# qianduoduolr/FGVC

Hardware: AMD Instinct MI355X
Metric: frames/sec + ms/corr-volume, 480p 8-frame clip, 1/2/4/8 MI355X (higher is better)
Workload: dtype f16 + fp6 (e2m3) MFMA operands, f32 accumulate; top-k near-ties re-scored in f64 from f32 features

## Files before the change

fgvc_amd/_lib.py:

```python
from __future__ import annotations

import ctypes as C
import contextlib
import os

_HERE = os.path.dirname(os.path.abspath(__file__))
LIB_PATH = os.environ.get("FGVC_HIP_LIB") or os.path.join(_HERE, "lib", "libfgvc_hip.so")

FGVC_OK = 0
ERR_INVALID_ARG, ERR_UNSUPPORTED, ERR_LAUNCH = 1, 2, 3
NO_LIMIT = 0x3FFFFFFF
PAIR_MASKED = 1
WEIGHT_SOFTMAX, WEIGHT_COSINE, WEIGHT_RAW = 0, 1, 2

_p = C.c_void_p
_i = C.c_int
_f = C.c_float

SIGNATURES = {
    "fgvc_version": (C.c_char_p, []),
    "fgvc_last_error": (C.c_char_p, []),
    "fgvc_set_option": (_i, [C.c_char_p, _i]),
    "fgvc_r2max_for_radius": (_i, [_f]),
    "fgvc_normalize_chw_to_hwc_f32": (_i, [_p, _p, _i, _i, _i, _i, _i, _p]),
    "fgvc_pair_topk_f32": (_i, [_p, _p, _p, _i, _i, _i, _i, _i, _i, _i, _i, _i, _i, _p, _p, _p, _p]),
    "fgvc_pair_topk_f16x3": (_i, [_p, _p, _p, _i, _i, _i, _i, _i, _i, _i, _i, _i, _i, _i, _p, _p, _p]),
    "fgvc_pair_topk_f16x3_runs": (_i, [_p, _p, _p, _i, _i, _i, _i, _i, _i, _i, _i, _i, _i, _i, _p, _i, _p, _p, _p]),
    "fgvc_split_f16x2": (_i, [_p, _p, C.c_int64, _i, _p]),
    "fgvc_split_f16f6p": (_i, [_p, _p, C.c_int64, _i, _p]),
    "fgvc_pair_topk_f16f6": (_i, [_p, _p, _p, _i, _i, _i, _i, _i, _i, _i, _i, _i, _i, _i, _p, _p, _p]),
    "fgvc_pair_topk_f16f6_runs": (_i, [_p, _p, _p, _i, _i, _i, _i, _i, _i, _i, _i, _i, _i, _i, _p, _i, _p, _p, _p]),
    "fgvc_split_f16f6x": (_i, [_p, _p, C.c_int64, _i, _p]),
    "fgvc_pair_topk_f16f6x": (_i, [_p, _p, _p, _i, _i, _i, _i, _i, _i, _i, _i, _i, _i, _i, _p, _p, _p]),
    "fgvc_pair_topk_f16f6x_runs": (_i, [_p, _p, _p, _i, _i, _i, _i, _i, _i, _i, _i, _i, _i, _i, _p, _i, _p, _p, _p]),
    "fgvc_merge_refine_workspace_bytes": (C.c_size_t, [_i, _i]),
    "fgvc_merge_refine_topk_f32": (_i, [_p, _p, _p, _p, _p, C.c_int64, _i, _p, C.c_int64, _i, _i, _i, _i, _i, _i, _i, _i, _i, _f, _i, _f, _i, _i, _i,
                                        _p, _p, _p, _p, _p]),
    "fgvc_pair_topk_f16x3_timed_out": (_i, []),
    "fgvc_pair_topk_f16x3_probe": (_i, [_p]),
    "fgvc_conv64_probe": (_i, [_p]),
    "fgvc_nchw_to_split_nhwc_f32": (_i, [_p, _p, _p, _i, _i, _i, _i, _i, _i, _p]),
    "fgvc_conv_split_f32": (_i, [_p, _p, _p, _p, _p, _p, _i, _i, _i, _i, _i, _i, _i, _i, _i, _p]),
    "fgvc_conv_split_fmt_f32": (_i, [_p, _p, _p, _p, _p, _p, _i, _i, _i, _i, _i, _i, _i, _i, _i, _i, _i, _i, _i, _p, _p]),
    "fgvc_conv_split_proj_fmt_f32": (_i, [_p, _p, _p, _p, _p, _p, _p, _p, _i, _i, _i, _i, _i, _i, _i, _i, _i, _i, _i, _i, _p, _p]),
    "fgvc_conv_split_bank_f16f6p_f32": (_i, [_p, _p, _p, _p, _p, _i, _i, _i, _i, _i, _i, _i, _i, _i, _i, _i, _p]),
    "fgvc_conv_split_bank_f16f6x_f32": (_i, [_p, _p, _p, _p, _p, _i, _i, _i, _i, _i, _i, _i, _i, _i, _i, _i, _p]),
    "fgvc_conv64_split_f32": (_i, [_p, _p, _p, _p, _p, _p, _i, _i, _i, _i, _i, _i, _p]),
    "fgvc_conv64_split_res_f32": (_i, [_p, _p, _p, _p, _p, _p, _p, _i, _i, _i, _i, _i, _i, _p]),
    "fgvc_conv64_split_fmt_f32": (_i, [_p, _p, _p, _p, _p, _p, _p, _i, _i, _i, _i, _i, _i, _i, _i, _i, _i, _p, _p]),
    "fgvc_conv_s2_split_f32": (_i, [_p, _p, _p, _p, _p, _i, _i, _i, _i, _i, _i, _i, _i, _i, _i, _i, _p]),
    "fgvc_conv_s2_split_fmt_f32": (_i, [_p, _p, _p, _p, _p, _i, _i, _i, _i, _i, _i, _i, _i, _i, _i, _i, _i, _i, _p, _p]),
    "fgvc_stem7_split_f32": (_i, [_p, _p, _p, _p, _p, _i, _i, _i, _i, _i, _i, _p]),
    "fgvc_stem7_split_fmt_f32": (_i, [_p, _p, _p, _p, _p, _i, _i, _i, _i, _i, _i, _i, _i, _p, _p]),
    "fgvc_nhwc_to_split_f32": (_i, [_p, _p, _i, _i, _i, _i, _i, _i, _i, _p]),
    "fgvc_normalize_nhwc_f32": (_i, [_p, _p, _i, _i, _i, _i, _i, _p]),
    "fgvc_normalize_split_nhwc_f32": (_i, [_p, _p, _p, _i, _i, _i, _i, _i, _p]),
    "fgvc_normalize_split_f16x2_nhwc_f32": (_i, [_p, _p, _p, _i, _i, _i, _i, _i, _p]),
    "fgvc_normalize_split_f16f6p_nhwc_f32": (_i, [_p, _p, _i, _i, _i, _i, _i, _p]),
    "fgvc_normalize_split_f16f6x_nhwc_f32": (_i, [_p, _p, _i, _i, _i, _i, _i, _p]),
    "fgvc_merge_topk_f32": (_i, [_p, _p, _p, _i, _i, _i, _i, _i, _f, _i, _p, _p, _p, _p]),
    "fgvc_propagate_topk_f32": (_i, [_p, _p, _i, _p, _p, _i, _i, _i, _i, _i, _i, _i, _p, _p]),
    "fgvc_corr_volume_f32": (_i, [_p, _p, _i, _i, _i, _f, _p, _p]),
    "fgvc_split_bf16": (_i, [_p, _p, C.c_int64, _i, _p]),
    "fgvc_corr_volume_bf16x3": (_i, [_p, _p, _i, _i, _i, _f, _p, _p]),
    "fgvc_corr_volume_bf16": (_i, [_p, _p, _i, _i, _i, _f, _p, _p]),
    "fgvc_split_f16f8": (_i, [_p, _p, C.c_int64, _i, _p]),
    "fgvc_corr_volume_f16f8": (_i, [_p, _p, _i, _i, _i, _f, _p, _p]),
    "fgvc_split_f16f6": (_i, [_p, _p, C.c_int64, _i, _p]),
    "fgvc_corr_volume_f16f6": (_i, [_p, _p, _i, _i, _i, _f, _p, _p]),
    "fgvc_debug_store_sweep_f32": (_i, [_p, C.c_int64, _i, _p]),
    "fgvc_dense_attend_splits": (_i, [_i, _i]),
    "fgvc_dense_attend_f32": (_i, [_p, _p, _i, _i, _i, _i, _i, _i, _i, _i, _i, _i, _i, _p, _i, _p]),
    "fgvc_dense_attend_finish_f32": (_i, [_p, _i, _i, _i, _i, _p, _p]),
    "fgvc_dense_kth_f32": (_i, [_p, _i, _i, _i, _p, _i, _p, _p]),
    "fgvc_dense_propagate_f32": (_i, [_p, _p, _i, _i, _i, _p, _p, _i, _p, _p]),
    "fgvc_local_corr_topk_f32": (_i, [_p, _p, _p, _i, _i, _i, _i, _i, _i, _f, _p, _p, _p, _p, _p, _p]),
    "fgvc_local_corr_topk_f16x3": (_i, [_p, _p, _p, _i, _i, _i, _i, _i, _i, _f, _p, _p, _p, _p, _p, _p]),
    "fgvc_local_merge_plan_f32": (_i, [_p, _p, _i, _p, _i, _i, _i, _i, _i, _i, _f, _p, _p, _p, _p]),
    "fgvc_topk_coord_f32": (_i, [_p, _p, _i, _i, _i, _i, _i, _p, _p]),
    "fgvc_topk_coord_rows_f32": (_i, [_p, _p, _i, _i, _i, _i, _i, _i, _p, _p]),
    "fgvc_cycle_chase_f32": (_i, [_p, _p, _p, _i, _i, _i, _i, _i, _p, _p, _p]),
    "fgvc_frames_rgb8_to_lab_f32": (_i, [_p, _i, _i, _i, C.c_int64, C.c_int64, C.c_int64, C.c_int64, _i, _i, _i, _i, _i, _i, _p, _p]),
    "fgvc_jf_tile_rows": (_i, []),
    "fgvc_jf_counts_u8": (_i, [_p, _p, _i, _i, _i, _i, _i, _p, _p]),
    "fgvc_render_frames_u8": (_i, [_p, C.c_int64, C.c_int64, _p, C.c_int64, C.c_int64, _i, _i, _i, _p, C.c_int64, C.c_int64, _p, _i, _i,
                                   _p, C.c_int64, C.c_int64, _p, C.c_int64, C.c_int64, _p, _i, _i, _p, _p]),
    "fgvc_render_tile_rows": (_i, []),
    "fgvc_render_tile_cols": (_i, []),
    "fgvc_c2f_refine_f32": (_i, [_p, _p, _p, _p, _i, _i, _i, _i, _i, _i, _i, _i, _f, _p, _p, _p, _p]),
    "fgvc_c2f_refine_mode_f32": (_i, [_p, _p, _p, _p, _i, _i, _i, _i, _i, _i, _i, _i, _f, _i, _p, _p, _p, _p]),
    "fgvc_bn_act_f32": (_i, [_p, _p, _p, _p, _p, _p, _f, _i, _p, _i, _i, _i, _p]),
    "fgvc_gaussian_labels_f32": (_i, [_p, _i, _i, _i, _i, _f, _p, _p]),
    "fgvc_softargmax_workspace_bytes": (C.c_size_t, [_i, _i]),
    "fgvc_softargmax_top5_f32": (_i, [_p, _i, _i, _i, _i, _i, _i, _p, _f, _p, _p, _p]),
    "fgvc_seg_max_label_u8": (_i, [_p, _i, _i, _i, _i, _p, _p]),
    "fgvc_seg_onehot_labels_u8": (_i, [_p, _i, _i, _i, _i, _i, _p, _p]),
    "fgvc_seg_hard_onehot_f32": (_i, [_p, _i, _i, _p, _p]),
    "fgvc_seg_readout_workspace_bytes": (C.c_size_t, [_i, _i]),
    "fgvc_seg_readout_u8": (_i, [_p, _i, _i, _i, _i, _i, _i, _i, _i, _i, _i, _i, _i, _i, _p, _p, _p]),
    "fgvc_seg_soft_labels_f32": (_i, [_p, _i, _i, _i, _i, _i, _i, _i, _i, _i, _p, _p]),
    "fgvc_seg_soft_labels_f64": (_i, [_p, _i, _i, _i, _i, _i, _i, _i, _i, _i, _p, _p]),
    "fgvc_heatmap_coords_workspace_bytes": (C.c_size_t, [_i, _i]),
    "fgvc_heatmap_coords_f32": (_i, [_p, _p, _i, _i, _i, _i, _i, _i, _i, _i, _i, _i, _i, _i, _i, _i, _p, _p, _p]),
    "fgvc_softmap_readout_f32": (_i, [_p, _p, _i, _i, _i, _i, _i, _i, _i, _i, _i, _i, _i, _i, _i, _i, _i, _i, _p, _p]),
}

_lib = None


class FgvcHipError(RuntimeError):
    pass


def load() -> C.CDLL:
    global _lib
    if _lib is None:
        import torch
        if not os.path.exists(LIB_PATH):
            raise FgvcHipError(
                f"{LIB_PATH} is missing: build it with `python -m fgvc_amd.build` "
                "(hipcc --offload-arch=gfx950). There is no CPU fallback.")
        lib = C.CDLL(LIB_PATH)
        for name, (res, args) in SIGNATURES.items():
            fn = getattr(lib, name)
            fn.restype, fn.argtypes = res, args
        _lib = lib
    return _lib


ABLATIONS_PATH = os.path.join(_HERE, "lib", "libfgvc_hip_ablations.so")
_ablations = None


@contextlib.contextmanager
def ablations():
    global _lib, _ablations
    prod = load()
    if _ablations is None:
        if not os.path.exists(ABLATIONS_PATH):
            raise FgvcHipError(f"{ABLATIONS_PATH} is missing: `python -m fgvc_amd.build` makes it beside the production library")
        lib = C.CDLL(ABLATIONS_PATH)
        for name, (res, args) in SIGNATURES.items():
            fn = getattr(lib, name)
            fn.restype, fn.argtypes = res, args
        _ablations = lib
    _lib = _ablations
    try:
        yield _ablations
    finally:
        _lib = prod


def call(name: str, *args) -> None:
    lib = load()
    rc = getattr(lib, name)(*args)
    if rc != FGVC_OK:
        raise FgvcHipError(f"{name} failed (code {rc}): {lib.fgvc_last_error().decode()}")
```

fgvc_amd/csrc/capi.hip:

```cpp
#include <stdarg.h>
#include <string.h>

#include "common.hpp"

namespace fgvc {

static thread_local char g_err[512] = "";

void set_error(const char* fmt, ...) {
  va_list ap;
  va_start(ap, fmt);
  vsnprintf(g_err, sizeof(g_err), fmt, ap);
  va_end(ap);
}

int pair_topk_launch(const float*, const float*, const int32_t*, int, int, int, int, int, int, int, int, int, int,
                     const uint8_t*, int32_t*, float*, hipStream_t);
int merge_topk_launch(const int32_t*, const float*, const int32_t*, int, int, int, int, int, float, int, int32_t*,
                      float*, float*, hipStream_t);
int normalize_launch(const float*, float*, int, int, int, int, int, hipStream_t);
int propagate_launch(const float*, const int32_t*, int, const int32_t*, const float*, int, int, int, int, int, int,
                     int, float*, hipStream_t);
int bn_act_launch(const float*, const float*, const float*, const float*, const float*, const float*, float, int, float*,
                  int, int, int, hipStream_t);
int gaussian_launch(const float*, int, int, int, int, float, float*, hipStream_t);
int softargmax_launch(const float*, int, int, int, int, int, int, const float*, float, double*, float*, hipStream_t);
int softargmax_bands();
int corr_volume_f32_launch(const float*, const float*, int, int, int, float, float*, hipStream_t);
int split_bf16_launch(const float*, uint16_t*, long long, int, hipStream_t);
int corr_volume_bf16_launch(const uint16_t*, const uint16_t*, int, int, int, float, float*, int, hipStream_t);
int local_merge_launch(const int32_t*, const float*, int, int, int, int, int, float, int32_t*, float*, float*,
                       hipStream_t);
int local_merge_plan_launch(const int32_t*, const float*, const int32_t*, int, int, int, int, int, int, int, float, int32_t*, float*,
                            float*, hipStream_t);
int topk_coord_launch(const int32_t*, const float*, int, int, int, int, int, float*, hipStream_t);
int topk_coord_rows_launch(const int32_t*, const float*, int, int, int, int, int, int, float*, hipStream_t);
int cycle_chase_launch(const float*, const float*, const float*, int, int, int, int, int, float*, float*, hipStream_t);
int frames_rgb8_to_lab_launch(const uint8_t*, int, int, int, long long, long long, long long, long long, int, int, int, int, int, int, float*,
                              hipStream_t);
int jf_counts_launch(const uint8_t*, const uint8_t*, int, int, int, int, int, int64_t*, hipStream_t);
int jf_tile_rows();
int render_frames_launch(const uint8_t*, long long, long long, uint8_t*, long long, long long, int, int, int, const uint8_t*, long long, long long,
                         const uint8_t*, int, int, const double*, long long, long long, const uint8_t*, long long, long long, const uint8_t*, int,
                         int, const double*, hipStream_t);
void render_tile(int*, int*);
int c2f_refine_launch(const int32_t*, const float*, const float*, const float*, int, int, int, int, int, int, int,
                      int, float, int, float*, int32_t*, float*, hipStream_t);

int conv_split_launch(const uint16_t*, const uint16_t*, const float*, const float*, uint16_t*, float*, int, int, int, int, int,
                      int, int, int, int, int, int, int, int, int*, hipStream_t, unsigned char* y_bank = nullptr, int bank_normalize = 1, const uint16_t* x2 = nullptr,
                      const uint16_t* w2 = nullptr, int Cin2 = 0, int bank_row_bytes = 1024);
int conv_s2_launch(const uint16_t*, const uint16_t*, const float*, uint16_t*, float*, int, int, int, int, int, int, int, int, int,
                   int, int, int, int, int*, hipStream_t);
int conv64_launch(const uint16_t*, const uint16_t*, const float*, const float*, const uint16_t*, uint16_t*, float*, int, int, int, int, int, int,
                  int, int, int, int, int*, hipStream_t);
int stem7_launch(const float*, const uint16_t*, const float*, uint16_t*, float*, int, int, int, int, int, int, int, int, int, int, int*,
                 hipStream_t);
int nchw_to_split_nhwc_launch(const float*, uint16_t*, float*, int, int, int, int, int, int, hipStream_t);
int normalize_nhwc_launch(const float*, float*, uint16_t*, int, int, int, int, int, int, hipStream_t);
int nhwc_to_split_launch(float*, uint16_t*, int, int, int, int, int, int, int, hipStream_t);

void set_conv_cot_cap(int);
void set_conv_narrow(int);
void set_conv64_variant(int);
int conv64_probe_read(long long*);
void set_conv_debug(int);
void set_corr6_skew(int);
void set_corr6_sdma(int);
void set_pair_debug(int);
void set_readout_prune(int);
void set_conv_s2_debug(int);
int split_f16x2_launch(const float*, uint16_t*, long long, int, hipStream_t);
int split_f16f6p_launch(const float*, unsigned char*, long long, int, hipStream_t);
int pair_topk_v7_launch(const uint16_t*, const uint16_t*, const int32_t*, int, int, int, int, int, int, int, int, int, const int32_t*, int,
                        int32_t*, float*, int, hipStream_t);
int pair_topk_v5_launch(const uint16_t*, const uint16_t*, const int32_t*, int, int, int, int, int, int, int, int, int, int, const int32_t*,
                        int, int32_t*, float*, hipStream_t);
void set_pair_v5_debug(int);
int pair_v5_timeout_flag();
int pair_v5_probe_read(long long*);
void set_corr_debug(int);
int split_f16f8_launch(const float*, unsigned char*, long long, int, hipStream_t);
int corr_volume_f16f8_launch(const unsigned char*, const unsigned char*, int, int, float, float*, hipStream_t);
void set_corr8_debug(int);
int split_f16f6_launch(const float*, unsigned char*, long long, hipStream_t);
int corr_volume_f16f6_launch(const unsigned char*, const unsigned char*, int, int, float, float*, hipStream_t);
void set_corr6_debug(int);
int store_sweep_launch(float*, long long, int, hipStream_t);
int dense_attend_splits(int, int);
int dense_attend_launch(const float*, const float*, int, int, int, int, int, int, int, int, int, int, int, float*, int, hipStream_t, const float*);
int dense_kth_launch(const float*, int, int, int, float*, int, float*, hipStream_t);
int dense_attend_finish_launch(const float*, int, int, int, int, float*, hipStream_t);

static bool aligned16(const void* p) { return (reinterpret_cast<uintptr_t>(p) & 15u) == 0; }

}

using namespace fgvc;

extern "C" {

const char* fgvc_version(void) { return "fgvc_hip 0.1 (gfx950)"; }
const char* fgvc_last_error(void) { return g_err; }

static int ablation_bits(const char* name, int value) {
  if (strcmp(name, "corr_debug") == 0 || strcmp(name, "pair_debug") == 0 || strcmp(name, "conv_s2_debug") == 0) return value;
  if (strcmp(name, "corr8_debug") == 0) return value & (1 | 2);
  if (strcmp(name, "corr6_debug") == 0) return value & (1 | 2 | 256 | 512 | 1024);
  if (strcmp(name, "conv_debug") == 0) return value & (1 | 2 | 4);
  if (strcmp(name, "pair_f16_debug") == 0)
    return value & ((value & 4194304) ? (1 | 2 | 524288 | 1048576) : (1 | 2 | 4 | 8 | 16 | 32 | 64 | 2048 | 524288 | 1048576));
  return 0;
}

int fgvc_set_option(const char* name, int value) {
  FGVC_REQUIRE(name != nullptr, FGVC_ERR_INVALID_ARG, "fgvc_set_option: null name");
#ifndef FGVC_ABLATIONS
  FGVC_REQUIRE(ablation_bits(name, value) == 0, FGVC_ERR_UNSUPPORTED,
               "fgvc_set_option: %s = %d switches a profiling ablation on (bits %d: results would be wrong); this library is built without them -- "
               "use libfgvc_hip_ablations.so (FGVC_HIP_LIB)", name, value, ablation_bits(name, value));
#endif
  if (strcmp(name, "corr_debug") == 0) {
    set_corr_debug(value);
    return FGVC_OK;
  }
  if (strcmp(name, "corr8_debug") == 0) {
    set_corr8_debug(value);
    return FGVC_OK;
  }
  if (strcmp(name, "corr6_debug") == 0) {
    set_corr6_debug(value);
    return FGVC_OK;
  }
  if (strcmp(name, "pair_debug") == 0) {
    set_pair_debug(value);
    return FGVC_OK;
  }
  if (strcmp(name, "corr6_sdma") == 0) {
    set_corr6_sdma(value);
    return FGVC_OK;
  }
  if (strcmp(name, "corr6_skew") == 0) {
    set_corr6_skew(value);
    return FGVC_OK;
  }
  if (strcmp(name, "conv_debug") == 0) {
    set_conv_debug(value);
    return FGVC_OK;
  }
  if (strcmp(name, "conv64_variant") == 0) {
    set_conv64_variant(value);
    return FGVC_OK;
  }
  if (strcmp(name, "conv_narrow") == 0) {
    set_conv_narrow(value);
    return FGVC_OK;
  }
  if (strcmp(name, "conv_cot_cap") == 0) {
    FGVC_REQUIRE(value == 0 || value == 64 || value == 128, FGVC_ERR_INVALID_ARG, "fgvc_set_option: conv_cot_cap must be 0, 64 or 128");
    set_conv_cot_cap(value);
    return FGVC_OK;
  }
  if (strcmp(name, "pair_f16_debug") == 0) {
    set_pair_v5_debug(value);
    return FGVC_OK;
  }
  if (strcmp(name, "conv_s2_debug") == 0) {
    set_conv_s2_debug(value);
    return FGVC_OK;
  }
  if (strcmp(name, "readout_prune") == 0) {
    set_readout_prune(value != 0);
    return FGVC_OK;
  }
  set_error("fgvc_set_option: unknown option '%s'", name);
  return FGVC_ERR_INVALID_ARG;
}

int fgvc_r2max_for_radius(float radius) {
  if (!(radius > 0.f)) return -1;
  long long d2 = (long long)ceil((double)radius * (double)radius) + 2;
  if (d2 > FGVC_NO_LIMIT) return FGVC_NO_LIMIT;
  while (d2 >= 0 && !(sqrtf((float)d2) < radius)) --d2;
  return (int)d2;
}

int fgvc_normalize_chw_to_hwc_f32(const float* in, float* out, int n, int C, int HW, int normalize, int c_out,
                                  void* stream) {
  FGVC_REQUIRE(in && out, FGVC_ERR_INVALID_ARG, "fgvc_normalize_chw_to_hwc_f32: null pointer");
  FGVC_REQUIRE(n >= 0 && C > 0 && HW > 0, FGVC_ERR_INVALID_ARG, "fgvc_normalize_chw_to_hwc_f32: bad shape n=%d C=%d HW=%d", n, C, HW);
  FGVC_REQUIRE(C <= 1024, FGVC_ERR_UNSUPPORTED, "fgvc_normalize_chw_to_hwc_f32: C=%d > 1024 (LDS tile)", C);
  FGVC_REQUIRE(n <= 65535, FGVC_ERR_UNSUPPORTED, "fgvc_normalize_chw_to_hwc_f32: n=%d > 65535 frames per call", n);
  FGVC_REQUIRE(c_out >= C, FGVC_ERR_INVALID_ARG, "fgvc_normalize_chw_to_hwc_f32: c_out=%d < C=%d", c_out, C);
  if (n == 0) return FGVC_OK;
  return normalize_launch(in, out, n, C, HW, normalize, c_out, (hipStream_t)stream);
}

int fgvc_pair_topk_f32(const float* qfeat, const float* kfeat, const int32_t* pairs, int n_pairs, int C, int Hq,
                       int Wq, int Hk, int Wk, int r2max, int ry, int rx, int topk, const uint8_t* dense_mask,
                       int32_t* idx_out, float* score_out, void* stream) {
  FGVC_REQUIRE(qfeat && kfeat && pairs && idx_out && score_out, FGVC_ERR_INVALID_ARG, "fgvc_pair_topk_f32: null pointer");
  FGVC_REQUIRE(aligned16(qfeat) && aligned16(kfeat) && aligned16(pairs), FGVC_ERR_INVALID_ARG,
               "fgvc_pair_topk_f32: qfeat/kfeat/pairs must be 16-byte aligned");
  FGVC_REQUIRE(Hq > 0 && Wq > 0 && Hk > 0 && Wk > 0 && n_pairs >= 0, FGVC_ERR_INVALID_ARG,
               "fgvc_pair_topk_f32: bad shape Hq=%d Wq=%d Hk=%d Wk=%d n_pairs=%d", Hq, Wq, Hk, Wk, n_pairs);
  FGVC_REQUIRE(topk >= 1 && topk <= 16, FGVC_ERR_UNSUPPORTED, "fgvc_pair_topk_f32: topk=%d outside 1..16", topk);
// ... 468 lines not shown
int fgvc_bn_act_f32(const float* x, const float* residual, const float* mean, const float* var, const float* gamma,
                    const float* beta, float eps, int relu, float* out, int N, int C, int HW, void* stream) {
  FGVC_REQUIRE(x && mean && var && gamma && beta && out, FGVC_ERR_INVALID_ARG, "fgvc_bn_act_f32: null pointer");
  FGVC_REQUIRE(N >= 0 && C > 0 && HW > 0 && eps >= 0.f, FGVC_ERR_INVALID_ARG, "fgvc_bn_act_f32: bad shape");
  if (N == 0) return FGVC_OK;
  return bn_act_launch(x, residual, mean, var, gamma, beta, eps, relu, out, N, C, HW, (hipStream_t)stream);
}

static bool conv_pad_ok(int H, int W, int Hp, int Wp) {
  return Hp >= 8 * cdiv(H, 8) + 2 && Wp >= 32 * cdiv(W, 32) + 8;
}

int fgvc_nchw_to_split_nhwc_f32(const float* in, uint16_t* out, float* out_f32, int N, int C, int H, int W, int Hp, int Wp,
                                void* stream) {
  FGVC_REQUIRE(in && (out || out_f32), FGVC_ERR_INVALID_ARG, "fgvc_nchw_to_split_nhwc_f32: null pointer");
  FGVC_REQUIRE(N >= 0 && C > 0 && C % 32 == 0 && H > 0 && W > 0, FGVC_ERR_INVALID_ARG,
               "fgvc_nchw_to_split_nhwc_f32: bad shape (C must be a multiple of 32)");
  FGVC_REQUIRE(conv_pad_ok(H, W, Hp, Wp), FGVC_ERR_INVALID_ARG,
               "fgvc_nchw_to_split_nhwc_f32: padded size %dx%d too small for %dx%d (need >= 8*ceil(H/8)+2 x 32*ceil(W/32)+8)", Hp, Wp, H, W);
  FGVC_REQUIRE(aligned16(out) && aligned16(out_f32) && (long long)N * (C / 32) <= 65535 && H <= 65535, FGVC_ERR_INVALID_ARG,
               "fgvc_nchw_to_split_nhwc_f32: alignment / grid limits");
  if (N == 0) return FGVC_OK;
  return nchw_to_split_nhwc_launch(in, out, out_f32, N, C, H, W, Hp, Wp, (hipStream_t)stream);
}

int fgvc_conv_split_f32(const uint16_t* x, const uint16_t* w, const float* bias, const float* residual, uint16_t* y_split,
                        float* y_f32, int N, int H, int W, int Hp, int Wp, int Cin, int Cout, int KS, int relu,
                        void* stream) {
  return fgvc_conv_split_fmt_f32(x, w, bias, residual, y_split, y_f32, N, H, W, Hp, Wp, Cin, Cout, KS, relu, FGVC_ACT_BF16X2, 0,
                                 FGVC_ACT_BF16X2, 0, nullptr, stream);
}

int fgvc_conv_split_fmt_f32(const uint16_t* x, const uint16_t* w, const float* bias, const float* residual, uint16_t* y_split,
                            float* y_f32, int N, int H, int W, int Hp, int Wp, int Cin, int Cout, int KS, int relu, int in_fmt,
                            int in_scale_log2, int out_fmt, int out_scale_log2, int* overflow, void* stream) {
  FGVC_REQUIRE(x && w && bias && (y_split || y_f32), FGVC_ERR_INVALID_ARG, "fgvc_conv_split_f32: null pointer");
  FGVC_REQUIRE(in_fmt >= 0 && in_fmt <= 3 && out_fmt >= 0 && out_fmt <= 3, FGVC_ERR_INVALID_ARG, "fgvc_conv_split_fmt_f32: unknown format %d / %d", in_fmt, out_fmt);
  FGVC_REQUIRE(out_fmt == FGVC_ACT_BF16X2 || !y_split || overflow, FGVC_ERR_INVALID_ARG, "fgvc_conv_split_fmt_f32: an f16-format output needs the overflow word");
  FGVC_REQUIRE(in_scale_log2 > -100 && in_scale_log2 < 100 && out_scale_log2 > -100 && out_scale_log2 < 100, FGVC_ERR_INVALID_ARG,
               "fgvc_conv_split_fmt_f32: scale exponent out of range");
  FGVC_REQUIRE(N >= 0 && H > 0 && W > 0, FGVC_ERR_INVALID_ARG, "fgvc_conv_split_f32: bad shape");
  FGVC_REQUIRE(KS == 1 || KS == 3, FGVC_ERR_UNSUPPORTED, "fgvc_conv_split_f32: kernel size %d (1 or 3, stride 1)", KS);
  FGVC_REQUIRE(Cin > 0 && Cin % 32 == 0 && Cout > 0 && Cout % 64 == 0, FGVC_ERR_UNSUPPORTED,
               "fgvc_conv_split_f32: Cin=%d must be a multiple of 32 and Cout=%d of 64", Cin, Cout);
  FGVC_REQUIRE(conv_pad_ok(H, W, Hp, Wp), FGVC_ERR_INVALID_ARG, "fgvc_conv_split_f32: padded size %dx%d too small for %dx%d", Hp, Wp, H, W);
  FGVC_REQUIRE(aligned16(x) && aligned16(w) && aligned16(bias) && aligned16(residual) && aligned16(y_split) && aligned16(y_f32),
               FGVC_ERR_INVALID_ARG, "fgvc_conv_split_f32: 16-byte alignment required");
  FGVC_REQUIRE((const void*)x != (const void*)y_split, FGVC_ERR_INVALID_ARG, "fgvc_conv_split_f32: in-place not supported");
  if (N == 0) return FGVC_OK;
  return conv_split_launch(x, w, bias, residual, y_split, y_f32, N, H, W, Hp, Wp, Cin, Cout, KS, relu, in_fmt, in_scale_log2, out_fmt,
                           out_scale_log2, overflow, (hipStream_t)stream);
}

int fgvc_conv_split_proj_fmt_f32(const uint16_t* x, const uint16_t* w, const uint16_t* x2, const uint16_t* w2, const float* bias,
                                 const float* residual, uint16_t* y_split, float* y_f32, int N, int H, int W, int Hp, int Wp, int Cin, int Cin2,
                                 int relu, int in_fmt, int in_scale_log2, int out_fmt, int out_scale_log2, int* overflow, void* stream) {
  FGVC_REQUIRE(x && w && x2 && w2 && bias && (y_split || y_f32), FGVC_ERR_INVALID_ARG, "fgvc_conv_split_proj_fmt_f32: null pointer");
  FGVC_REQUIRE(in_fmt >= 0 && in_fmt <= 3 && out_fmt >= 0 && out_fmt <= 3, FGVC_ERR_INVALID_ARG, "fgvc_conv_split_proj_fmt_f32: unknown format %d / %d", in_fmt, out_fmt);
  FGVC_REQUIRE(out_fmt == FGVC_ACT_BF16X2 || !y_split || overflow, FGVC_ERR_INVALID_ARG, "fgvc_conv_split_proj_fmt_f32: an f16-format output needs the overflow word");
  FGVC_REQUIRE(in_scale_log2 > -100 && in_scale_log2 < 100 && out_scale_log2 > -100 && out_scale_log2 < 100, FGVC_ERR_INVALID_ARG,
               "fgvc_conv_split_proj_fmt_f32: scale exponent out of range");
  FGVC_REQUIRE(N >= 0 && H > 0 && W > 0, FGVC_ERR_INVALID_ARG, "fgvc_conv_split_proj_fmt_f32: bad shape");
  FGVC_REQUIRE(Cin > 0 && Cin % 32 == 0 && Cin2 > 0 && Cin2 % 32 == 0, FGVC_ERR_UNSUPPORTED,
               "fgvc_conv_split_proj_fmt_f32: Cin=%d and Cin2=%d must be multiples of 32 (Cout is 256)", Cin, Cin2);
  FGVC_REQUIRE(conv_pad_ok(H, W, Hp, Wp), FGVC_ERR_INVALID_ARG, "fgvc_conv_split_proj_fmt_f32: padded size %dx%d too small for %dx%d", Hp, Wp, H, W);
  FGVC_REQUIRE(aligned16(x) && aligned16(w) && aligned16(x2) && aligned16(w2) && aligned16(bias) && aligned16(residual) && aligned16(y_split) &&
               aligned16(y_f32), FGVC_ERR_INVALID_ARG, "fgvc_conv_split_proj_fmt_f32: 16-byte alignment required");
  FGVC_REQUIRE((const void*)x != (const void*)y_split && (const void*)x2 != (const void*)y_split, FGVC_ERR_INVALID_ARG,
               "fgvc_conv_split_proj_fmt_f32: in-place not supported");
  if (N == 0) return FGVC_OK;
  return conv_split_launch(x, w, bias, residual, y_split, y_f32, N, H, W, Hp, Wp, Cin, 256, 3, relu, in_fmt, in_scale_log2, out_fmt,
                           out_scale_log2, overflow, (hipStream_t)stream, nullptr, 1, x2, w2, Cin2);
}

static int conv_split_bank_common(const uint16_t* x, const uint16_t* w, const float* bias, const float* residual, void* bank, int N,
                                  int H, int W, int Hp, int Wp, int Cin, int KS, int relu, int in_fmt, int in_scale_log2,
                                  int normalize, void* stream, int row_bytes) {
  FGVC_REQUIRE(x && w && bias && bank, FGVC_ERR_INVALID_ARG, "fgvc_conv_split_bank_f16f6p_f32: null pointer");
  FGVC_REQUIRE(in_fmt >= 0 && in_fmt <= 3, FGVC_ERR_INVALID_ARG, "fgvc_conv_split_bank_f16f6p_f32: unknown format %d", in_fmt);
  FGVC_REQUIRE(in_scale_log2 > -100 && in_scale_log2 < 100, FGVC_ERR_INVALID_ARG, "fgvc_conv_split_bank_f16f6p_f32: scale exponent out of range");
  FGVC_REQUIRE(N >= 0 && H > 0 && W > 0, FGVC_ERR_INVALID_ARG, "fgvc_conv_split_bank_f16f6p_f32: bad shape");
  FGVC_REQUIRE(KS == 3, FGVC_ERR_UNSUPPORTED, "fgvc_conv_split_bank_f16f6p_f32: kernel size %d (3 x 3, stride 1: the last convolution of a BasicBlock)", KS);
  FGVC_REQUIRE(Cin > 0 && Cin % 32 == 0, FGVC_ERR_UNSUPPORTED, "fgvc_conv_split_bank_f16f6p_f32: Cin=%d must be a multiple of 32 (Cout is 256)", Cin);
  FGVC_REQUIRE(conv_pad_ok(H, W, Hp, Wp), FGVC_ERR_INVALID_ARG, "fgvc_conv_split_bank_f16f6p_f32: padded size %dx%d too small for %dx%d", Hp, Wp, H, W);
  FGVC_REQUIRE(aligned16(x) && aligned16(w) && aligned16(bias) && aligned16(residual) && aligned16(bank), FGVC_ERR_INVALID_ARG,
               "fgvc_conv_split_bank_f16f6p_f32: 16-byte alignment required");
  if (N == 0) return FGVC_OK;
  return conv_split_launch(x, w, bias, residual, nullptr, nullptr, N, H, W, Hp, Wp, Cin, 256, KS, relu, in_fmt, in_scale_log2, 0, 0, nullptr,
                           (hipStream_t)stream, reinterpret_cast<unsigned char*>(bank), normalize, nullptr, nullptr, 0, row_bytes);
}

int fgvc_conv_split_bank_f16f6p_f32(const uint16_t* x, const uint16_t* w, const float* bias, const float* residual, void* bank, int N,
                                    int H, int W, int Hp, int Wp, int Cin, int KS, int relu, int in_fmt, int in_scale_log2,
                                    int normalize, void* stream) {
  return conv_split_bank_common(x, w, bias, residual, bank, N, H, W, Hp, Wp, Cin, KS, relu, in_fmt, in_scale_log2, normalize, stream, 1024);
}

int fgvc_conv_split_bank_f16f6x_f32(const uint16_t* x, const uint16_t* w, const float* bias, const float* residual, void* bank, int N,
                                    int H, int W, int Hp, int Wp, int Cin, int KS, int relu, int in_fmt, int in_scale_log2,
                                    int normalize, void* stream) {
  return conv_split_bank_common(x, w, bias, residual, bank, N, H, W, Hp, Wp, Cin, KS, relu, in_fmt, in_scale_log2, normalize, stream, 2048);
}

int fgvc_conv64_probe(int64_t* out32) {
  FGVC_REQUIRE(out32 != nullptr, FGVC_ERR_INVALID_ARG, "fgvc_conv64_probe: null pointer");
  return conv64_probe_read(reinterpret_cast<long long*>(out32)) == 0 ? FGVC_OK : FGVC_ERR_LAUNCH;
}

int fgvc_conv64_split_f32(const uint16_t* x, const uint16_t* w, const float* bias, const float* residual, uint16_t* y_split,
                          float* y_f32, int N, int H, int W, int Hp, int Wp, int relu, void* stream) {
  return fgvc_conv64_split_res_f32(x, w, bias, residual, nullptr, y_split, y_f32, N, H, W, Hp, Wp, relu, stream);
}

int fgvc_conv64_split_res_f32(const uint16_t* x, const uint16_t* w, const float* bias, const float* residual,
                              const uint16_t* residual_split, uint16_t* y_split, float* y_f32, int N, int H, int W, int Hp, int Wp,
                              int relu, void* stream) {
  return fgvc_conv64_split_fmt_f32(x, w, bias, residual, residual_split, y_split, y_f32, N, H, W, Hp, Wp, relu, FGVC_ACT_BF16X2, 0,
                                   FGVC_ACT_BF16X2, 0, nullptr, stream);
}

int fgvc_conv64_split_fmt_f32(const uint16_t* x, const uint16_t* w, const float* bias, const float* residual,
                              const uint16_t* residual_split, uint16_t* y_split, float* y_f32, int N, int H, int W, int Hp, int Wp,
                              int relu, int in_fmt, int in_scale_log2, int out_fmt, int out_scale_log2, int* overflow, void* stream) {
  FGVC_REQUIRE(x && w && bias && (y_split || y_f32), FGVC_ERR_INVALID_ARG, "fgvc_conv64_split_f32: null pointer");
  FGVC_REQUIRE((in_fmt == FGVC_ACT_BF16X2 || in_fmt == FGVC_ACT_F16F8) && (out_fmt == FGVC_ACT_BF16X2 || out_fmt == FGVC_ACT_F16F8),
               FGVC_ERR_UNSUPPORTED, "fgvc_conv64_split_fmt_f32: formats %d -> %d (bf16x2 or f16f8)", in_fmt, out_fmt);
  FGVC_REQUIRE(out_fmt == FGVC_ACT_BF16X2 || !y_split || overflow, FGVC_ERR_INVALID_ARG,
               "fgvc_conv64_split_fmt_f32: an f16-format output needs the overflow word");
  FGVC_REQUIRE(in_scale_log2 > -100 && in_scale_log2 < 100 && out_scale_log2 > -100 && out_scale_log2 < 100, FGVC_ERR_INVALID_ARG,
               "fgvc_conv64_split_fmt_f32: scale exponent out of range");
  FGVC_REQUIRE(!(residual && residual_split), FGVC_ERR_INVALID_ARG, "fgvc_conv64_split_res_f32: one residual, f32 or split, not both");
  FGVC_REQUIRE(!residual_split || in_fmt == FGVC_ACT_BF16X2, FGVC_ERR_UNSUPPORTED,
               "fgvc_conv64_split_fmt_f32: a split residual is read as (hi, lo) bf16: bf16x2 tensors only");
  FGVC_REQUIRE(N >= 0 && H > 0 && W > 0, FGVC_ERR_INVALID_ARG, "fgvc_conv64_split_f32: bad shape");
  FGVC_REQUIRE(conv_pad_ok(H, W, Hp, Wp), FGVC_ERR_INVALID_ARG, "fgvc_conv64_split_f32: padded size %dx%d too small for %dx%d", Hp, Wp, H, W);
  FGVC_REQUIRE(aligned16(x) && aligned16(w) && aligned16(bias) && aligned16(residual) && aligned16(residual_split) && aligned16(y_split) &&
                   aligned16(y_f32),
               FGVC_ERR_INVALID_ARG, "fgvc_conv64_split_f32: 16-byte alignment required");
  FGVC_REQUIRE((const void*)x != (const void*)y_split && (!residual_split || (const void*)residual_split != (const void*)y_split),
               FGVC_ERR_INVALID_ARG, "fgvc_conv64_split_f32: in-place not supported");
  if (N == 0) return FGVC_OK;
  return conv64_launch(x, w, bias, residual, residual_split, y_split, y_f32, N, H, W, Hp, Wp, relu, in_fmt, in_scale_log2, out_fmt,
                       out_scale_log2, overflow, (hipStream_t)stream);
}

int fgvc_conv_s2_split_f32(const uint16_t* x, const uint16_t* w, const float* bias, uint16_t* y_split, float* y_f32, int N,
                           int H, int W, int Hp, int Wp, int Cin, int Cout, int KS, int Hop, int Wop, int relu, void* stream) {
  return fgvc_conv_s2_split_fmt_f32(x, w, bias, y_split, y_f32, N, H, W, Hp, Wp, Cin, Cout, KS, Hop, Wop, relu, FGVC_ACT_BF16X2, 0, nullptr, stream);
}

int fgvc_conv_s2_split_fmt_f32(const uint16_t* x, const uint16_t* w, const float* bias, uint16_t* y_split, float* y_f32, int N,
                               int H, int W, int Hp, int Wp, int Cin, int Cout, int KS, int Hop, int Wop, int relu, int out_fmt,
                               int out_scale_log2, int* overflow, void* stream) {
  FGVC_REQUIRE(x && w && bias && (y_split || y_f32), FGVC_ERR_INVALID_ARG, "fgvc_conv_s2_split_f32: null pointer");
  FGVC_REQUIRE(out_fmt >= 0 && out_fmt <= 3 && out_scale_log2 > -100 && out_scale_log2 < 100, FGVC_ERR_INVALID_ARG, "fgvc_conv_s2_split_fmt_f32: bad output format / scale");
  FGVC_REQUIRE(out_fmt == FGVC_ACT_BF16X2 || !y_split || overflow, FGVC_ERR_INVALID_ARG, "fgvc_conv_s2_split_fmt_f32: an f16-format output needs the overflow word");
  FGVC_REQUIRE(N >= 0 && H > 0 && W > 0, FGVC_ERR_INVALID_ARG, "fgvc_conv_s2_split_f32: bad shape");
  FGVC_REQUIRE(KS == 1 || KS == 3, FGVC_ERR_UNSUPPORTED, "fgvc_conv_s2_split_f32: kernel size %d (1 or 3, stride 2)", KS);
  FGVC_REQUIRE(Cin > 0 && Cin % 32 == 0 && Cout > 0 && Cout % 32 == 0, FGVC_ERR_UNSUPPORTED,
               "fgvc_conv_s2_split_f32: Cin=%d and Cout=%d must be multiples of 32", Cin, Cout);
  const int Ho = (H - 1) / 2 + 1, Wo = (W - 1) / 2 + 1;
  FGVC_REQUIRE(conv_pad_ok(H, W, Hp, Wp), FGVC_ERR_INVALID_ARG, "fgvc_conv_s2_split_f32: padded size %dx%d too small for %dx%d", Hp, Wp, H, W);
  FGVC_REQUIRE(!y_split || conv_pad_ok(Ho, Wo, Hop, Wop), FGVC_ERR_INVALID_ARG,
               "fgvc_conv_s2_split_f32: padded output size %dx%d too small for %dx%d", Hop, Wop, Ho, Wo);
  FGVC_REQUIRE(aligned16(x) && aligned16(w) && aligned16(bias) && aligned16(y_split) && aligned16(y_f32),
               FGVC_ERR_INVALID_ARG, "fgvc_conv_s2_split_f32: 16-byte alignment required");
  FGVC_REQUIRE((const void*)x != (const void*)y_split, FGVC_ERR_INVALID_ARG, "fgvc_conv_s2_split_f32: in-place not supported");
  if (N == 0) return FGVC_OK;
  return conv_s2_launch(x, w, bias, y_split, y_f32, N, Hp, Wp, Cin, Cout, KS, Ho, Wo, Hop, Wop, relu, out_fmt, out_scale_log2, overflow,
                        (hipStream_t)stream);
}

int fgvc_stem7_split_f32(const float* x, const uint16_t* w, const float* bias, uint16_t* y_split, float* y_f32, int N, int H,
                         int W, int Hop, int Wop, int relu, void* stream) {
  return fgvc_stem7_split_fmt_f32(x, w, bias, y_split, y_f32, N, H, W, Hop, Wop, relu, FGVC_ACT_BF16X2, 0, nullptr, stream);
}

int fgvc_stem7_split_fmt_f32(const float* x, const uint16_t* w, const float* bias, uint16_t* y_split, float* y_f32, int N, int H,
                             int W, int Hop, int Wop, int relu, int out_fmt, int out_scale_log2, int* overflow, void* stream) {
  FGVC_REQUIRE(x && w && bias && (y_split || y_f32), FGVC_ERR_INVALID_ARG, "fgvc_stem7_split_f32: null pointer");
  FGVC_REQUIRE(out_fmt == FGVC_ACT_BF16X2 || out_fmt == FGVC_ACT_F16F8, FGVC_ERR_UNSUPPORTED, "fgvc_stem7_split_fmt_f32: output format %d", out_fmt);
  FGVC_REQUIRE(out_fmt == FGVC_ACT_BF16X2 || !y_split || overflow, FGVC_ERR_INVALID_ARG,
               "fgvc_stem7_split_fmt_f32: an f16-format output needs the overflow word");
  FGVC_REQUIRE(out_scale_log2 > -100 && out_scale_log2 < 100, FGVC_ERR_INVALID_ARG, "fgvc_stem7_split_fmt_f32: scale exponent out of range");
  FGVC_REQUIRE(N >= 0 && H > 0 && W > 0, FGVC_ERR_INVALID_ARG, "fgvc_stem7_split_f32: bad shape");
  const int Ho = (H - 1) / 2 + 1, Wo = (W - 1) / 2 + 1;
  FGVC_REQUIRE(!y_split || conv_pad_ok(Ho, Wo, Hop, Wop), FGVC_ERR_INVALID_ARG,
               "fgvc_stem7_split_f32: padded output size %dx%d too small for %dx%d", Hop, Wop, Ho, Wo);
  FGVC_REQUIRE(aligned16(w) && aligned16(bias) && aligned16(y_split) && aligned16(y_f32) && ((uintptr_t)x & 3) == 0,
               FGVC_ERR_INVALID_ARG, "fgvc_stem7_split_f32: alignment (16 bytes; 4 for x)");
  if (N == 0) return FGVC_OK;
  return stem7_launch(x, w, bias, y_split, y_f32, N, H, W, Ho, Wo, Hop, Wop, relu, out_fmt, out_scale_log2, overflow, (hipStream_t)stream);
}

int fgvc_nhwc_to_split_f32(float* x, uint16_t* out, int N, int C, int H, int W, int Hp, int Wp, int relu, void* stream) {
  FGVC_REQUIRE(x && out, FGVC_ERR_INVALID_ARG, "fgvc_nhwc_to_split_f32: null pointer");
  FGVC_REQUIRE(N >= 0 && C > 0 && C % 32 == 0 && H > 0 && W > 0, FGVC_ERR_INVALID_ARG,
               "fgvc_nhwc_to_split_f32: bad shape (C must be a multiple of 32)");
  FGVC_REQUIRE(conv_pad_ok(H, W, Hp, Wp), FGVC_ERR_INVALID_ARG, "fgvc_nhwc_to_split_f32: padded size %dx%d too small for %dx%d", Hp, Wp, H, W);
  FGVC_REQUIRE(aligned16(x) && aligned16(out), FGVC_ERR_INVALID_ARG, "fgvc_nhwc_to_split_f32: 16-byte alignment required");
  FGVC_REQUIRE((long long)N * H * W * C / 4 < (1ll << 31) * 256, FGVC_ERR_UNSUPPORTED, "fgvc_nhwc_to_split_f32: tensor too large");
  if (N == 0) return FGVC_OK;
  return nhwc_to_split_launch(x, out, N, C, H, W, Hp, Wp, relu, (hipStream_t)stream);
}

static int normalize_split_common(const char* what, const float* in, float* out_f32, uint16_t* out_split, int N, int C, int H, int W,
                                  int normalize, int fmt, void* stream) {
  FGVC_REQUIRE(in && (out_f32 || out_split), FGVC_ERR_INVALID_ARG, "%s: null pointer", what);
  FGVC_REQUIRE(N >= 0 && C > 0 && C % 4 == 0 && H > 0 && W > 0, FGVC_ERR_INVALID_ARG, "%s: bad shape", what);
  FGVC_REQUIRE(aligned16(in) && aligned16(out_f32) && aligned16(out_split), FGVC_ERR_INVALID_ARG, "%s: 16-byte alignment required", what);
  if (N == 0) return FGVC_OK;
  return normalize_nhwc_launch(in, out_f32, out_split, N, C, H, W, normalize, fmt, (hipStream_t)stream);
}

int fgvc_normalize_split_nhwc_f32(const float* in, float* out_f32, uint16_t* out_split, int N, int C, int H, int W, int normalize,
                                  void* stream) {
  return normalize_split_common("fgvc_normalize_split_nhwc_f32", in, out_f32, out_split, N, C, H, W, normalize, 0, stream);
}

int fgvc_normalize_split_f16x2_nhwc_f32(const float* in, float* out_f32, uint16_t* out_split, int N, int C, int H, int W,
                                        int normalize, void* stream) {
  return normalize_split_common("fgvc_normalize_split_f16x2_nhwc_f32", in, out_f32, out_split, N, C, H, W, normalize, 1, stream);
}

int fgvc_normalize_split_f16f6p_nhwc_f32(const float* in, uint8_t* rows, int N, int C, int H, int W, int normalize, void* stream) {
  FGVC_REQUIRE(C == 256, FGVC_ERR_UNSUPPORTED, "fgvc_normalize_split_f16f6p_nhwc_f32: C=%d unsupported (256 only)", C);
  return normalize_split_common("fgvc_normalize_split_f16f6p_nhwc_f32", in, nullptr, reinterpret_cast<uint16_t*>(rows), N, C, H, W, normalize, 2, stream);
}

int fgvc_normalize_split_f16f6x_nhwc_f32(const float* in, uint8_t* rows, int N, int C, int H, int W, int normalize, void* stream) {
  FGVC_REQUIRE(C == 256, FGVC_ERR_UNSUPPORTED, "fgvc_normalize_split_f16f6x_nhwc_f32: C=%d unsupported (256 only)", C);
  return normalize_split_common("fgvc_normalize_split_f16f6x_nhwc_f32", in, nullptr, reinterpret_cast<uint16_t*>(rows), N, C, H, W, normalize, 3, stream);
}

int fgvc_normalize_nhwc_f32(const float* in, float* out, int N, int C, int H, int W, int normalize, void* stream) {
  FGVC_REQUIRE(in && out, FGVC_ERR_INVALID_ARG, "fgvc_normalize_nhwc_f32: null pointer");
  return fgvc_normalize_split_nhwc_f32(in, out, nullptr, N, C, H, W, normalize, stream);
}

int fgvc_gaussian_labels_f32(const float* points, int P, int Hf, int Wf, int stride, float sigma, float* out,
                             void* stream) {
  FGVC_REQUIRE(points && out, FGVC_ERR_INVALID_ARG, "fgvc_gaussian_labels_f32: null pointer");
  FGVC_REQUIRE(P > 0 && Hf > 0 && Wf > 0 && stride >= 1 && sigma > 0.f, FGVC_ERR_INVALID_ARG, "fgvc_gaussian_labels_f32: bad shape");
  return gaussian_launch(points, P, Hf, Wf, stride, sigma, out, (hipStream_t)stream);
}

size_t fgvc_softargmax_workspace_bytes(int n_frames, int P) {
  if (n_frames < 0 || P < 0) return 0;
  return (size_t)n_frames * P * (softargmax_bands() * (2 * 5 + 1) + 1) * sizeof(float);
}

int fgvc_softargmax_top5_f32(const float* labels, int n_frames, int Hf, int Wf, int P, int h, int w,
                             const float* gauss_points, float sigma, double* coords, void* workspace, void* stream) {
  FGVC_REQUIRE(labels && coords, FGVC_ERR_INVALID_ARG, "fgvc_softargmax_top5_f32: null pointer");
  FGVC_REQUIRE(n_frames >= 0 && Hf > 0 && Wf > 0 && P > 0 && h > 0 && w > 0, FGVC_ERR_INVALID_ARG, "fgvc_softargmax_top5_f32: bad shape");
  FGVC_REQUIRE((long long)h * w < (1ll << 31) && h * w >= 5, FGVC_ERR_UNSUPPORTED, "fgvc_softargmax_top5_f32: h*w out of range");
  FGVC_REQUIRE(n_frames <= 65535 && sigma > 0.f, FGVC_ERR_INVALID_ARG, "fgvc_softargmax_top5_f32: bad n_frames/sigma");
  FGVC_REQUIRE(workspace != nullptr || n_frames == 0, FGVC_ERR_INVALID_ARG,
               "fgvc_softargmax_top5_f32: workspace of fgvc_softargmax_workspace_bytes() bytes required");
  FGVC_REQUIRE(P <= 65535, FGVC_ERR_UNSUPPORTED, "fgvc_softargmax_top5_f32: P > 65535");
  if (n_frames == 0) return FGVC_OK;
  return softargmax_launch(labels, n_frames, Hf, Wf, P, h, w, gauss_points, sigma, coords,
                           static_cast<float*>(workspace), (hipStream_t)stream);
}

}
```

fgvc_amd/csrc/conv_s2.hip:

```cpp
#include "common.hpp"

namespace fgvc {

struct ConvS2Params {
  const uint16_t* x;
  const uint16_t* w;
  const float* bias;
  uint16_t* y_split;
  float* y_f32;
  int N, Hp, Wp, Cin, Cout, Ho, Wo, Hop, Wop, relu;
  int n_ty, n_tx;
  int debug;
  float out_scale;
  int out_fmt;
  int* overflow;
};


__device__ __forceinline__ void s2_lds_dma_16(const void* src_lane, uint32_t lds_uniform) {
  asm volatile("s_mov_b32 m0, %1\n\ts_nop 0\n\tglobal_load_lds_dwordx4 %0, off" ::"v"(src_lane), "s"(lds_uniform) : "memory");
}
__device__ __forceinline__ uint32_t s2_lds_addr(const void* p) {
  return (uint32_t)(size_t)(const __attribute__((address_space(3))) unsigned char*)p;
}
__device__ __forceinline__ int s2_swz(int e, int s) { return e * 128 + ((s ^ ((e >> 1) & 7)) << 4); }

constexpr int S2_TR = 4;
constexpr int S2_NW = 2 * S2_TR;
constexpr int S2_CPG = 1;
constexpr int S2_RS = 144;

template <int KS>
__global__ __launch_bounds__(64 * S2_NW, 2) void conv_s2_kernel(ConvS2Params p) {
  constexpr int T = KS * KS;
  constexpr int NR = KS == 3 ? 2 * S2_TR + 1 : S2_TR;
  constexpr int NC = KS == 3 ? 65 : 32;
  constexpr int NE = NR * NC;
  constexpr int NG = (NE + 7) / 8;
  constexpr int CHUNKB = NG * 8 * 128;
  constexpr int SMEMB = S2_CPG * CHUNKB > S2_NW * 32 * S2_RS ? S2_CPG * CHUNKB : S2_NW * 32 * S2_RS;
  static_assert(SMEMB <= 79 * 1024, "LDS: two workgroups per CU");
  __shared__ __attribute__((aligned(16))) unsigned char smem[SMEMB];
  auto wave_sync = [&]() { asm volatile("s_waitcnt lgkmcnt(0)" ::: "memory"); };

  const int tid = threadIdx.x, lane = tid & 63;
  const int wave = __builtin_amdgcn_readfirstlane(tid >> 6);
  const int ct = wave & 3, half = wave >> 2;
  const int n = lane & 31, h = lane >> 5;
  int bid = blockIdx.x;
  const int nimg = bid / (p.n_ty * p.n_tx);
  bid -= nimg * p.n_ty * p.n_tx;
  const int ty = bid / p.n_tx, tx = bid - ty * p.n_tx;
  const int y0 = ty * S2_TR, x0 = tx * 32;
  const int co_w = blockIdx.y * 128 + ct * 32;
  const bool active = co_w < p.Cout;
  const int nchunk = p.Cin / 32;
  const size_t pix_bytes_in = (size_t)nchunk * 128;
  const int d_row = lane >> 3, d_slot = lane & 7;

  f32x16 acc[2];
#pragma unroll
  for (int b = 0; b < 2; ++b)
#pragma unroll
    for (int r = 0; r < 16; ++r) acc[b][r] = 0.f;

  const int n_ct = p.Cout / 32;
  const uint16_t* wlane = p.w + (size_t)(active ? (co_w >> 5) : 0) * 2048 + lane * 8;
  f32x4 bias_v[4];
#pragma unroll
  for (int g = 0; g < 4; ++g) bias_v[g] = *reinterpret_cast<const f32x4*>(p.bias + (active ? co_w : 0) + 8 * g + 4 * h);

  for (int cg = 0; cg < nchunk; cg += S2_CPG) {
    const int ncg = imin(S2_CPG, nchunk - cg);
    for (int i = wave; i < ((p.debug & 1) ? 0 : ncg * NG); i += S2_NW) {
      const int cc = i / NG, g = i - cc * NG;
      const int e = imin(g * 8 + d_row, NE - 1);
      const int j = e / NC, m = e - j * NC;
      int prow, pcol;
      if (KS == 3) {
        prow = 2 * y0 + j;
        pcol = 2 * x0 + (m < 33 ? 2 * m : 2 * (m - 33) + 1);
      } else {
        prow = 2 * (y0 + j) + 1;
        pcol = 2 * (x0 + m) + 1;
      }
      if (prow >= p.Hp || pcol >= p.Wp) prow = pcol = 0;
      const int sl = d_slot ^ ((e >> 1) & 7);
      const unsigned char* src = reinterpret_cast<const unsigned char*>(p.x) +
                                 (((size_t)nimg * p.Hp + prow) * p.Wp + pcol) * pix_bytes_in + (size_t)(cg + cc) * 128 + sl * 16;
      s2_lds_dma_16(src, s2_lds_addr(smem + cc * CHUNKB + g * 1024));
    }
    asm volatile("s_waitcnt vmcnt(0)" ::: "memory");
    __syncthreads();

    const int nit = ncg * T;
    bf16x8 a_cur[4], a_nxt[4];
    auto load_a = [&](bf16x8* a, int it) {
      const int cc = it / T, t = it - cc * T;
      const uint16_t* wp = wlane + ((size_t)t * nchunk + (cg + cc)) * n_ct * 2048;
#pragma unroll
      for (int q = 0; q < 4; ++q) a[q] = *reinterpret_cast<const bf16x8*>((p.debug & 8) ? wlane + q * 512 : wp + q * 512);
    };
    load_a(a_cur, 0);
    for (int it = 0; it < nit; ++it) {
      if (it + 1 < nit) load_a(a_nxt, it + 1);
      __builtin_amdgcn_sched_barrier(0);
      const int cc = it / T, t = it - cc * T;
      const int dy = KS == 3 ? t / 3 : 0, dx = KS == 3 ? t - 3 * (t / 3) : 0;
      const int mbase = KS == 3 ? (dx == 0 ? 0 : dx == 1 ? 33 : 1) : 0;
      const unsigned char* patch = smem + cc * CHUNKB;
#pragma unroll
      for (int b = 0; b < 2; ++b) {
        const int r = half * 2 + b;
        const int e = (KS == 3 ? (2 * r + dy) : r) * NC + mbase + n;
        bf16x8 xh[2], xl[2];
#pragma unroll
        for (int s = 0; s < 2; ++s) {
          xh[s] = *reinterpret_cast<const bf16x8*>(patch + s2_swz(e, 2 * s + h));
          xl[s] = *reinterpret_cast<const bf16x8*>(patch + s2_swz(e, 4 + 2 * s + h));
        }
        if (p.debug & 2) {
          acc[b][0] += (float)(xh[0][0] + xl[0][0] + xh[1][0] + xl[1][0] + a_cur[0][0] + a_cur[1][0] + a_cur[2][0] + a_cur[3][0]);
          continue;
        }
#pragma unroll
        for (int s = 0; s < 2; ++s) {
          acc[b] = __builtin_amdgcn_mfma_f32_32x32x16_bf16(a_cur[s], xh[s], acc[b], 0, 0, 0);
          acc[b] = __builtin_amdgcn_mfma_f32_32x32x16_bf16(a_cur[2 + s], xh[s], acc[b], 0, 0, 0);
          acc[b] = __builtin_amdgcn_mfma_f32_32x32x16_bf16(a_cur[s], xl[s], acc[b], 0, 0, 0);
        }
      }
#pragma unroll
      for (int q = 0; q < 4; ++q) a_cur[q] = a_nxt[q];
    }
    __syncthreads();
  }
  if (!active || (p.debug & 4)) return;

  unsigned char* tile = smem + wave * (32 * S2_RS);
  const int mv_row = lane >> 3, mv_col = (lane & 7) * 16;
#pragma unroll
  for (int b = 0; b < 2; ++b) {
    const int y = y0 + half * 2 + b;
    if (y >= p.Ho) continue;
    f32x4 v[4];
#pragma unroll
    for (int g = 0; g < 4; ++g) {
      const f32x4 bv = bias_v[g];
      v[g] = {acc[b][4 * g + 0] + bv.x, acc[b][4 * g + 1] + bv.y, acc[b][4 * g + 2] + bv.z, acc[b][4 * g + 3] + bv.w};
      if (p.relu) {
        v[g].x = fmaxf(v[g].x, 0.f); v[g].y = fmaxf(v[g].y, 0.f); v[g].z = fmaxf(v[g].z, 0.f); v[g].w = fmaxf(v[g].w, 0.f);
      }
    }
    if (p.y_f32) {
#pragma unroll
      for (int g = 0; g < 4; ++g) *reinterpret_cast<f32x4*>(tile + n * S2_RS + (8 * g + 4 * h) * 4) = v[g];
      wave_sync();
      unsigned char* dst = reinterpret_cast<unsigned char*>(p.y_f32 + (((size_t)nimg * p.Ho + y) * p.Wo + x0) * p.Cout + co_w);
#pragma unroll
      for (int i = 0; i < 4; ++i) {
        const int row = i * 8 + mv_row;
        if (x0 + row < p.Wo)
          *reinterpret_cast<uint4*>(dst + (size_t)row * p.Cout * 4 + mv_col) =
              *reinterpret_cast<const uint4*>(tile + row * S2_RS + mv_col);
      }
      wave_sync();
    }
    if (p.y_split) {
      if (p.out_fmt == 0) {
#pragma unroll
        for (int g = 0; g < 4; ++g) {
          const f32x4 x = v[g];
          ushort4 hv, lv;
          split_bf16_4(x, hv, lv);
          unsigned char* o = tile + n * S2_RS + (8 * g + 4 * h) * 2;
          *reinterpret_cast<ushort4*>(o) = hv;
          *reinterpret_cast<ushort4*>(o + 64) = lv;
        }
      } else if (p.out_fmt == 3) {
        bool ovf = false;
        uint2 hw[4];
        fgvc_i32x4 main6, tail6;
        split_f16f6_chunk(v, p.out_scale, h, hw, main6, tail6, ovf);
        unsigned char* o = tile + n * S2_RS;
#pragma unroll
        for (int g = 0; g < 4; ++g) *reinterpret_cast<uint2*>(o + (8 * g + 4 * h) * 2) = hw[g];
        *reinterpret_cast<fgvc_i32x4*>(o + 80 - 16 * h) = main6;
        *reinterpret_cast<fgvc_i32x4*>(o + 112 - 16 * h) = tail6;
        if (__builtin_amdgcn_ballot_w64(ovf && x0 + n < p.Wo) != 0ull && lane == 0) atomicOr(p.overflow, 1);
      } else {
        bool ovf = false;
#pragma unroll
        for (int g = 0; g < 4; ++g) {
          uint2 hw, lw;
          uint32_t l8, h8;
          split_f16_4(v[g], p.out_scale, hw, l8, h8, lw, ovf);
          unsigned char* o = tile + n * S2_RS;
          *reinterpret_cast<uint2*>(o + (8 * g + 4 * h) * 2) = hw;
          if (p.out_fmt == 1) {
            *reinterpret_cast<uint32_t*>(o + 64 + 8 * g + 4 * h) = l8;
            *reinterpret_cast<uint32_t*>(o + 96 + 8 * g + 4 * h) = h8;
          } else {
            *reinterpret_cast<uint2*>(o + 64 + (8 * g + 4 * h) * 2) = lw;
          }
        }
        if (__builtin_amdgcn_ballot_w64(ovf && x0 + n < p.Wo) != 0ull && lane == 0) atomicOr(p.overflow, 1);
      }
      wave_sync();
      const size_t pix0 = ((size_t)nimg * p.Hop + (y + 1)) * p.Wop + (x0 + 1);
      unsigned char* dst = reinterpret_cast<unsigned char*>(p.y_split) + (pix0 * (p.Cout / 32) + (co_w >> 5)) * 128;
#pragma unroll
      for (int i = 0; i < 4; ++i) {
        const int row = i * 8 + mv_row;
        if (x0 + row < p.Wo)
          *reinterpret_cast<uint4*>(dst + (size_t)row * p.Cout * 4 + mv_col) =
              *reinterpret_cast<const uint4*>(tile + row * S2_RS + mv_col);
      }
      wave_sync();
    }
  }
}

static int g_conv_s2_debug = 0;
void set_conv_s2_debug(int v) { g_conv_s2_debug = v; }

int conv_s2_launch(const uint16_t* x, const uint16_t* w, const float* bias, uint16_t* y_split, float* y_f32, int N, int Hp,
                   int Wp, int Cin, int Cout, int KS, int Ho, int Wo, int Hop, int Wop, int relu, int out_fmt, int out_scale_log2,
                   int* overflow, hipStream_t s) {
  ConvS2Params p;
  p.out_fmt = out_fmt; p.out_scale = ldexpf(1.0f, out_scale_log2); p.overflow = overflow;
  p.x = x; p.w = w; p.bias = bias; p.y_split = y_split; p.y_f32 = y_f32;
  p.N = N; p.Hp = Hp; p.Wp = Wp; p.Cin = Cin; p.Cout = Cout; p.Ho = Ho; p.Wo = Wo; p.Hop = Hop; p.Wop = Wop; p.relu = relu;
  p.n_ty = cdiv(Ho, S2_TR); p.n_tx = cdiv(Wo, 32);
  p.debug = g_conv_s2_debug;
  dim3 grid(p.n_ty * p.n_tx * N, cdiv(Cout, 128));
  if (KS == 3) conv_s2_kernel<3><<<grid, 64 * S2_NW, 0, s>>>(p);
  else conv_s2_kernel<1><<<grid, 64 * S2_NW, 0, s>>>(p);
  FGVC_CHECK_LAUNCH("fgvc_conv_s2_split_f32");
  return FGVC_OK;
}

}
```

fgvc_amd/mmpt_api/backbones.py:

```python
from __future__ import annotations

import re
from typing import Sequence

import torch
import torch.nn as nn
import torch.nn.functional as F

from .registry import BACKBONES

_CAPTURING = [False]


class ConvBN(nn.Module):

    def __init__(self, cin, cout, k, stride=1, padding=0, dilation=1, relu=True):
        super().__init__()
        self.conv = nn.Conv2d(cin, cout, k, stride, padding, dilation, bias=False)
        self.bn = nn.BatchNorm2d(cout)
        self.relu = relu

    def forward(self, x, residual=None, relu=None):
        relu = self.relu if relu is None else relu
        y = self.conv(x)
        if y.is_cuda and not self.training and y.dtype == torch.float32 and y.is_contiguous():
            from .. import ops
            return ops.bn_act(y, self.bn, residual, relu, inplace=True)
        y = self.bn(y)
        if residual is not None:
            y = y + residual
        return F.relu(y, inplace=True) if relu else y


class BasicBlock(nn.Module):
    expansion = 1

    def __init__(self, cin, planes, stride=1, dilation=1, downsample=None):
        super().__init__()
        self.conv1 = ConvBN(cin, planes, 3, stride, dilation, dilation, relu=True)
        self.conv2 = ConvBN(planes, planes, 3, 1, 1, 1, relu=False)
        self.downsample = downsample

    def forward(self, x):
        idt = x if self.downsample is None else self.downsample(x)
        return self.conv2(self.conv1(x), residual=idt, relu=True)


class Bottleneck(nn.Module):
    expansion = 4

    def __init__(self, cin, planes, stride=1, dilation=1, downsample=None):
        super().__init__()
        self.conv1 = ConvBN(cin, planes, 1, 1, 0, 1, relu=True)
        self.conv2 = ConvBN(planes, planes, 3, stride, dilation, dilation, relu=True)
        self.conv3 = ConvBN(planes, planes * 4, 1, 1, 0, 1, relu=False)
        self.downsample = downsample

    def forward(self, x):
        idt = x if self.downsample is None else self.downsample(x)
        return self.conv3(self.conv2(self.conv1(x)), residual=idt, relu=True)


def _stage(block, cin, planes, n, stride, dilation):
    ds = None
    if stride != 1 or cin != planes * block.expansion:
        ds = ConvBN(cin, planes * block.expansion, 1, stride, 0, 1, relu=False)
    first_dil = dilation if dilation == 1 else dilation // 2
    layers = [block(cin, planes, stride, first_dil, ds)]
    layers += [block(planes * block.expansion, planes, 1, dilation) for _ in range(1, n)]
    return nn.Sequential(*layers)


@BACKBONES.register_module()
class ResNet(nn.Module):
    arch_settings = {18: (BasicBlock, (2, 2, 2, 2)), 34: (BasicBlock, (3, 4, 6, 3)),
                     50: (Bottleneck, (3, 4, 6, 3)), 101: (Bottleneck, (3, 4, 23, 3)),
                     152: (Bottleneck, (3, 8, 36, 3))}

    def __init__(self, depth, pretrained=None, torchvision_pretrain=True, in_channels=3, num_stages=4,
                 strides=(1, 2, 2, 2), dilations=(1, 1, 1, 1), out_indices=(3,), planes_custom=None,
                 pool_type="max", zero_init_residual=True, **unused):
        super().__init__()
        if depth not in self.arch_settings:
            raise KeyError(f"invalid depth {depth} for resnet")
        assert 1 <= num_stages <= 4 and len(strides) == len(dilations) == num_stages
        assert max(out_indices) < num_stages
        self.depth, self.pretrained, self.torchvision_pretrain = depth, pretrained, torchvision_pretrain
        self.strides, self.dilations, self.out_indices = tuple(strides), tuple(dilations), tuple(out_indices)
        self.zero_init_residual = zero_init_residual
        block, counts = self.arch_settings[depth]
        self.conv1 = ConvBN(in_channels, 64, 7, 2, 3, 1, relu=True)
        self.pool = {"max": nn.MaxPool2d(3, 2, 1), "mean": nn.AvgPool2d(3, 2, 1)}.get(pool_type)
        cin = 64
        self.res_layers = []
        for i, n in enumerate(counts[:num_stages]):
            planes = planes_custom[i] if planes_custom is not None else 64 * 2 ** i
            self.add_module(f"layer{i + 1}", _stage(block, cin, planes, n, strides[i], dilations[i]))
            self.res_layers.append(f"layer{i + 1}")
            cin = planes * block.expansion
        self.feat_dim = cin

    def init_weights(self):
        self.reset_split_cache()
        if isinstance(self.pretrained, (str, dict)):
            if self.torchvision_pretrain:
                load_torchvision_checkpoint(self, self.pretrained)
            elif isinstance(self.pretrained, str):
                load_checkpoint(self, self.pretrained)
            else:
                raise Exception("a state dict is only accepted as a torchvision checkpoint (resnet.py:590)")
            return
        for m in self.modules():
            if isinstance(m, nn.Conv2d):
                nn.init.kaiming_normal_(m.weight, mode="fan_out", nonlinearity="relu")
            elif isinstance(m, nn.BatchNorm2d):
                nn.init.constant_(m.weight, 1)
                nn.init.constant_(m.bias, 0)
        if self.zero_init_residual:
            for m in self.modules():
                if isinstance(m, BasicBlock):
                    nn.init.constant_(m.conv2.bn.weight, 0)
                elif isinstance(m, Bottleneck):
                    nn.init.constant_(m.conv3.bn.weight, 0)

    use_conv64 = True
    use_stem7 = True
    use_s2_conv = True
    conv64_f16f8 = True
    res_from_split = False
    use_split_conv = True
    arith = "f16f6"
    fold_projection = True
    layer1_whole_batch = True
    fuse_bank = True

    @staticmethod
    def supported_arith():
        return ("f16f6", "f16f8", "bf16x3", "f16x3")

    def set_arith(self, arith: str):
        if arith not in self.supported_arith():
            raise ValueError(f"arith={arith!r}: one of {self.supported_arith()}")
        if arith != self.arith:
            self.arith = arith
            self.reset_split_cache()

    def _generic_s1(self, cb) -> bool:
        c = cb.conv
        return c.stride == (1, 1) and not (self.use_conv64 and tuple(c.weight.shape) == (64, 64, 3, 3))

    def _is_conv64(self, cb) -> bool:
        c = cb.conv
        return bool(self.use_conv64 and c.stride == (1, 1) and tuple(c.weight.shape) == (64, 64, 3, 3))

    def _stem7_ok(self) -> bool:
        c1 = self.conv1.conv
        return bool(self.use_stem7 and c1.kernel_size == (7, 7) and c1.stride == (2, 2) and c1.padding == (3, 3) and c1.in_channels == 3
                    and c1.out_channels == 64 and c1.dilation == (1, 1) and self.conv1.relu)

    def _format_plan(self, last: int):
        from .. import ops
        fmt, bf = ops.ACT_FMT[self.arith], ops.ACT_BF16X2
        cache = self.__dict__.setdefault("_split_cache", {})
        key = ("fmt_plan", self.arith, last, self.use_conv64, self.use_s2_conv, self.use_stem7, self.conv64_f16f8)
        if key not in cache:
            blocks = [(s_i, b_i, blk) for s_i in range(last + 1) for b_i, blk in enumerate(getattr(self, self.res_layers[s_i]))]
            f64 = ops.ACT_F16F8 if (fmt in (ops.ACT_F16F8, ops.ACT_F16F6) and self.conv64_f16f8) else bf

            def reads(cb):
                if self._is_conv64(cb):
                    return f64
                return fmt if self._generic_s1(cb) else bf

            def can_write(cb, f):
                if f == bf:
                    return True
                if self._is_conv64(cb):
                    return f == ops.ACT_F16F8
                return self._generic_s1(cb) or (cb.conv.stride == (2, 2) and self.use_s2_conv)

            def wants(blk):
                f = reads(blk.conv1)
                return f if (blk.downsample is None or reads(blk.downsample) == f) else bf
            plan = {}
            f_in = wants(blocks[0][2]) if blocks else bf
            if f_in != bf and not (self._stem7_ok() and f_in == ops.ACT_F16F8):
                f_in = bf
            plan["stem"] = f_in
            for i, (s_i, b_i, blk) in enumerate(blocks):
                f_a = reads(blk.conv2) if can_write(blk.conv1, reads(blk.conv2)) else bf
                nxt = blocks[i + 1][2] if i + 1 < len(blocks) else None
                f_y = wants(nxt) if (nxt is not None and can_write(blk.conv2, wants(nxt))) else bf
                plan[(s_i, b_i)] = (f_in, f_a, f_y)
                f_in = f_y
            cache[key] = plan
        return cache[key]

    def _block_formats(self, si: int, bi: int, last: int):
        return self._format_plan(last)[(si, bi)]


    def _projection_fold(self, blk, wt, si, bi, dev, f_in, f_a, s_in, s_a, Cout, banked):
        from .. import ops
        ds, c2 = blk.downsample, blk.conv2
        if not (self.fold_projection and not banked and f_in == f_a and f_a != ops.ACT_F16F8 and wt["c2"][3] == "s1" and wt["ds"] is not None
                and wt["ds"][3] == "s1" and Cout == 256 and c2.conv.kernel_size == (3, 3) and ds.conv.kernel_size == (1, 1)
                and ds.conv.stride == (1, 1) and ds.conv.in_channels % 32 == 0):
            return None
        cache = self.__dict__.setdefault("_split_cache", {})
        e = s_a + wt["c2"][2] - s_in
        key = ("wproj", si, bi, dev, self.arith, f_a, e)
        if key not in cache:
            w = ds.conv.weight.detach()
            if f_a == ops.ACT_BF16X2:
                w2, b2 = ops.prepare_conv_split(w, ds.bn)
            else:
                sc = (ds.bn.weight / torch.sqrt(ds.bn.running_var + ds.bn.eps)).detach().float().abs().view(-1, 1, 1, 1)
                top = float((w.detach().float().abs() * sc).max()) * 2.0 ** e
                if not (2.0 ** -6 <= top < 2.0 ** 14) and top != 0.0:
                    cache[key] = None
                    return None
                w2, b2, _ = ops.prepare_conv_split_f16(w, ds.bn, f_a, force_exp=e)
            cache[key] = (w2, (wt["c2"][1] + b2).contiguous())
        return cache[key]

    def _identity_from_split(self, blk) -> bool:
        c2 = getattr(blk, "conv2", None)
        return bool(self.use_conv64 and self.res_from_split and not (self.arith in ("f16f8", "f16f6") and self.conv64_f16f8)
                    and isinstance(blk, BasicBlock) and blk.downsample is None
                    and c2 is not None and tuple(c2.conv.weight.shape) == (64, 64, 3, 3) and c2.conv.stride == (1, 1)
                    and tuple(blk.conv1.conv.weight.shape) == (64, 64, 3, 3) and blk.conv1.conv.stride == (1, 1))

    def _scales(self, dev):
        cache = self.__dict__.setdefault("_split_cache", {})
        return cache.get(("scales", dev))

    calibration = "canonical"
    CANON_TARGET_LOG2 = 8

    @staticmethod
    def canonical_frames(device):
        g = torch.Generator().manual_seed(0x5CA1E)
        base = torch.randn(2, 3, 24, 24, generator=g)
        x = F.interpolate(base, size=(192, 192), mode="bilinear", align_corners=False) * 1.5 + 0.4 * torch.randn(2, 3, 192, 192, generator=g)
        return x.clamp_(-2.7, 2.7).to(device)

    def calibrate(self, x=None, last=None, device=None):
        from .. import ops
        cache = self.__dict__.setdefault("_split_cache", {})
        canonical = x is None
        if canonical:
            x = self.canonical_frames(device if device is not None else next(self.parameters()).device)
        dev = x.device
        saved = (self.arith, self.split_lanes)
        rec = {}
        self.__dict__["_calib"] = rec
        try:
            self.arith, self.split_lanes = "bf16x3", 1
            self._trunk(x, max(self.out_indices) if last is None else last)
            torch.cuda.synchronize(dev)
        finally:
            self.arith, self.split_lanes = saved
            self.__dict__.pop("_calib", None)
        target = (self.CANON_TARGET_LOG2 if canonical else ops.F16_TARGET_LOG2) - int(self.__dict__.get("_headroom_extra", 0))
        scales = {k: ops.act_scale_log2(float(v), target) for k, v in rec.items()}
        cache[("scales", dev)] = scales
        cache[("scales_from", dev)] = "canonical" if canonical else "frames"
        self._drop_graphs(dev)
        if ("overflow", dev) not in cache:
            cache[("overflow", dev)] = torch.zeros(1, dtype=torch.int32, device=dev)
        self._cache_filled(dev)
        return scales

    def check_overflow(self):
        cache = self.__dict__.get("_split_cache", {})
        hit = False
        for k in [k for k in cache if isinstance(k, tuple) and k and k[0] == "overflow"]:
            if int(cache[k].item()) != 0:
                hit = True
                cache[k].zero_()
                cache.pop(("scales", k[1]), None)
                self._drop_graphs(k[1])
        if hit and self.calibration == "canonical":
            self.__dict__["_headroom_extra"] = min(int(self.__dict__.get("_headroom_extra", 0)) + 4, 12)
        return hit
# ... 13 lines not shown
            if shape_sig is not None and not (k[1][0] == shape_sig[0] and tuple(k[1][2:]) == tuple(shape_sig[1:3]) and k[2] == shape_sig[3]):
                continue
            del cache[k]

    def _load_from_state_dict(self, *args, **kwargs):
        self.__dict__.pop("_split_cache", None)
        return super()._load_from_state_dict(*args, **kwargs)

    def reset_split_cache(self):
        self.__dict__.pop("_split_cache", None)

    def _split_stage_ok(self, stage, x) -> bool:
        if not (self.use_split_conv and x.is_cuda and not self.training and x.dtype == torch.float32):
            return False
        for bi, blk in enumerate(stage):
            if not isinstance(blk, BasicBlock):
                return False
            convs = [blk.conv1.conv, blk.conv2.conv] + ([blk.downsample.conv] if blk.downsample is not None else [])
            for c in convs:
                if (c.dilation != (1, 1) or c.groups != 1 or c.in_channels % 32 or c.out_channels % 64
                        or c.kernel_size not in ((1, 1), (3, 3))):
                    return False
            strided = blk.conv1.conv.stride != (1, 1)
            if blk.conv2.conv.stride != (1, 1) or (strided and (bi > 0 or blk.downsample is None)):
                return False
            if blk.downsample is not None and blk.downsample.conv.stride != blk.conv1.conv.stride:
                return False
            if blk.downsample is None and blk.conv1.conv.in_channels != blk.conv2.conv.out_channels:
                return False
        return True

    def _split_buffers(self, key, N, C, H, W, device, names):
        from .. import ops
        cache = self.__dict__.setdefault("_split_cache", {})
        k = ("b", self.__dict__.get("_ws_sig")) + key + (N, C, H, W, device)
        mk = {"s": ops.alloc_split_nhwc, "f": ops.alloc_nhwc}
        if k not in cache:
            cache[k] = {}
        missing = [nm for nm in names if nm not in cache[k]]
        if missing:
            for nm in missing:
                cache[k][nm] = mk[nm[0]](N, C, H, W, device)
            self._cache_filled(device)
        return cache[k]

    max_workspace_shapes = 2

    def _touch_workspace_shape(self, sig):
        cache = self.__dict__.setdefault("_split_cache", {})
        order = cache.setdefault("_ws_order", [])
        if sig in order:
            order.remove(sig)
        order.append(sig)
        while len(order) > max(1, int(self.max_workspace_shapes)):
            old = order.pop(0)
            if _CAPTURING[0]:
                raise RuntimeError("ResNet: a workspace eviction inside a HIP-graph capture (the graph would keep freed addresses)")
            if isinstance(sig[-1], torch.device) and sig[-1].type == "cuda":
                torch.cuda.synchronize(sig[-1])
            self._drop_graphs(shape_sig=old)
            for k in [k for k in cache if isinstance(k, tuple) and len(k) > 1 and k[0] == "b" and k[1] == old]:
                del cache[k]
        self.__dict__["_ws_sig"] = sig

    @staticmethod
    def _cache_filled(device):
        if _CAPTURING[0]:
            raise RuntimeError("ResNet: a cache entry was made inside a HIP-graph capture (the capture call must find everything in place)")
        torch.cuda.synchronize(device)

    @staticmethod
    def _fold(cb: "ConvBN"):
        bn = cb.bn
        scale = (bn.weight / torch.sqrt(bn.running_var + bn.eps)).detach()
        w = (cb.conv.weight.detach() * scale.view(-1, 1, 1, 1)).contiguous(memory_format=torch.channels_last)
        return w, (bn.bias - bn.running_mean * scale).detach().contiguous()

    def _miopen_nhwc(self, key, cb: "ConvBN", x_cl):
        cache = self.__dict__.setdefault("_split_cache", {})
        k = ("m",) + key + (x_cl.device,)
        if k not in cache:
            cache[k] = self._fold(cb)
            self._cache_filled(x_cl.device)
        w, b = cache[k]
        c = cb.conv
        y = F.conv2d(x_cl, w, b, c.stride, c.padding, c.dilation, c.groups)
        y = y.contiguous(memory_format=torch.channels_last)
        return y.permute(0, 2, 3, 1)

    split_lanes = 2

    def _stage_split(self, si: int, cur, call):
        from .. import ops
        stage = getattr(self, self.res_layers[si])
        cache = self.__dict__.setdefault("_split_cache", {})
        dev = cur["split"].device
        lo, hi, N = cur["lo"], cur["hi"], cur["N"]
        from ..ops import ACT_BF16X2
        last_stage = call["last"]
        fmts = [self._block_formats(si, bi, last_stage) for bi in range(len(stage))]
        calib = self.__dict__.get("_calib")
        scales = self._scales(dev) or {}
        ovf = cache.get(("overflow", dev))
        wkey = ("w", si, dev, self.arith)
        if wkey not in cache:
            def prep_s1(w, bn, fmt):
                if self.use_conv64 and tuple(w.shape) == (64, 64, 3, 3):
                    if fmt == ops.ACT_F16F8:
                        return ops.prepare_conv64_f16(w, bn) + ("conv64",)
                    assert fmt == ACT_BF16X2
                    return ops.prepare_conv64(w, bn) + (0, "conv64")
                if fmt == ACT_BF16X2:
                    return ops.prepare_conv_split(w, bn) + (0, "s1")
                return ops.prepare_conv_split_f16(w, bn, fmt) + ("s1",)

            def prep(cb, fmt):
                st = cb.conv.stride
                if st == (1, 1):
                    return prep_s1(cb.conv.weight.detach(), cb.bn, fmt)
                if st == (2, 2):
                    return ops.prepare_conv_s2(cb.conv.weight.detach(), cb.bn) + (0, "s2")
                return None
            cache[wkey] = [dict(c1=prep(b.conv1, f[0]), c2=prep(b.conv2, f[1]),
                                ds=None if b.downsample is None else prep(b.downsample, f[0]))
                           for b, f in zip(stage, fmts)]
            self._cache_filled(dev)
        full = None
        for bi, (blk, wt) in enumerate(zip(stage, cache[wkey])):
            Cout = blk.conv2.conv.out_channels
            idt_split = None
            H, W = cur["H"], cur["W"]
            f_in, f_a, f_y = fmts[bi]
            s_in = cur.get("scale", 0)
            s_a = scales.get((si, bi, "a"), 0) if f_a != ACT_BF16X2 else 0
            s_y = scales.get((si, bi, "y"), 0) if f_y != ACT_BF16X2 else 0
            assert cur.get("fmt", ACT_BF16X2) == f_in, "split activation format mismatch between producer and consumer"

            def conv_s1(x_split, wb, in_fmt=ACT_BF16X2, in_scale=0, out_fmt=ACT_BF16X2, out_scale=0, **kw):
                if wb[3] == "conv64":
                    ops.conv64_split(x_split, wb[0], wb[1], H, W, in_fmt=in_fmt, in_scale_log2=in_scale + wb[2], out_fmt=out_fmt,
                                     out_scale_log2=out_scale, overflow=ovf, **kw)
                else:
                    ops.conv_split(x_split, wb[0], wb[1], H, W, in_fmt=in_fmt, in_scale_log2=in_scale + wb[2], out_fmt=out_fmt,
                                   out_scale_log2=out_scale, overflow=ovf, **kw)

            last_conv = bi == len(stage) - 1 and not cur["need_split"]
            proj = None
            x_in_split = cur["split"]
            if blk.conv1.conv.stride == (2, 2) and self.use_s2_conv:
                Hi, Wi = H, W
                H, W = (Hi - 1) // 2 + 1, (Wi - 1) // 2 + 1
                bufs = self._split_buffers((si, bi), N, Cout, H, W, dev, ("s_a", "s_y", "f_y", "f_idt"))
                buf = {k: v[lo:hi] for k, v in bufs.items()}
                ops.conv_s2_split(cur["split"], wt["ds"][0], wt["ds"][1], Hi, Wi, relu=False, out_f32=buf["f_idt"])
                idt = buf["f_idt"]
                ops.conv_s2_split(cur["split"], wt["c1"][0], wt["c1"][1], Hi, Wi, relu=True, out_split=buf["s_a"], out_fmt=f_a,
                                  out_scale_log2=s_a, overflow=ovf)
            elif blk.conv1.conv.stride != (1, 1):
                x_cl = cur["f32"].permute(0, 3, 1, 2)
                t1 = self._miopen_nhwc((si, bi, "c1"), blk.conv1, x_cl)
                idt = self._miopen_nhwc((si, bi, "ds"), blk.downsample, x_cl)
                _, H, W, _ = t1.shape
                bufs = self._split_buffers((si, bi), N, Cout, H, W, dev, ("s_a", "s_y", "f_y"))
                buf = {k: v[lo:hi] for k, v in bufs.items()}
                assert f_a == ACT_BF16X2
                ops.nhwc_to_split(t1, buf["s_a"], relu=True)
            else:
                bufs = self._split_buffers((si, bi), N, Cout, H, W, dev, ("s_a", "s_y", "f_y", "f_idt"))
                buf = {k: v[lo:hi] for k, v in bufs.items()}
                if blk.downsample is not None:
                    proj = self._projection_fold(blk, wt, si, bi, dev, f_in, f_a, s_in, s_a, Cout, last_conv and si == call["last"] and call.get("bank_of") is not None)
                if proj is not None:
                    idt = None
                elif blk.downsample is not None:
                    conv_s1(cur["split"], wt["ds"], f_in, s_in, relu=False, out_f32=buf["f_idt"])
                    idt = buf["f_idt"]
                elif self._identity_from_split(blk):
                    idt, idt_split = None, cur["split"]
                else:
                    idt = cur["f32"]
                    assert idt is not None
                conv_s1(cur["split"], wt["c1"], f_in, s_in, f_a, s_a, relu=True, out_split=buf["s_a"])
            if calib is not None:
                calib[(si, bi, "a")] = torch.maximum(calib.get((si, bi, "a"), torch.zeros((), device=dev)),
                                                     buf["s_a"].view(torch.bfloat16)[..., :32].abs().amax().float())
            full = bufs["f_y"]
            if bi == len(stage) - 1 and si in call["fresh"]:
                if si not in call["out"]:
                    with torch.cuda.stream(call["main"]):
                        call["out"][si] = ops.alloc_nhwc(N, Cout, H, W, dev)
                    for st in call["streams"]:
                        if st is not call["main"]:
                            st.wait_stream(call["main"])
                full = call["out"][si]
            f_y_ = full[lo:hi]
            skip_f32 = (not cur["need_f32"]) if bi == len(stage) - 1 else self._identity_from_split(stage[bi + 1])
            if skip_f32:
                f_y_ = None
            kw_res = dict(residual_split=idt_split) if idt_split is not None else dict(residual=idt)
            bank = None
            if (last_conv and si == call["last"] and call.get("bank_of") is not None and wt["c2"][3] == "s1" and Cout == 256
                    and blk.conv2.conv.kernel_size == (3, 3) and idt_split is None and calib is None):
                bank = call["bank_of"](lo, hi, Cout, H, W)
            if bank is not None:
                ops.conv_split_to_bank(buf["s_a"], wt["c2"][0], wt["c2"][1], H, W, True, bank, residual=idt, in_fmt=f_a,
                                       in_scale_log2=s_a + wt["c2"][2], normalize=call["bank_normalize"])
                cur = dict(cur, split=None, f32=None, H=H, W=W, fmt=f_y, scale=s_y, banked=True)
                continue
            if proj is not None:
                ops.conv_split(buf["s_a"], wt["c2"][0], proj[1], H, W, True, out_split=None if last_conv else buf["s_y"], out_f32=f_y_,
                               in_fmt=f_a, in_scale_log2=s_a + wt["c2"][2], out_fmt=f_y, out_scale_log2=s_y, overflow=ovf,
                               x2_split=x_in_split, w2=proj[0])
            else:
                conv_s1(buf["s_a"], wt["c2"], f_a, s_a, f_y, s_y, relu=True, out_split=None if last_conv else buf["s_y"], out_f32=f_y_, **kw_res)
            if calib is not None and not last_conv:
                calib[(si, bi, "y")] = torch.maximum(calib.get((si, bi, "y"), torch.zeros((), device=dev)),
                                                     buf["s_y"].view(torch.bfloat16)[..., :32].abs().amax().float())
            cur = dict(cur, split=buf["s_y"], f32=f_y_, H=H, W=W, fmt=f_y, scale=s_y)
        cur["full"] = full
        return cur

    def _trunk(self, x, last: int, fresh=(), post=None, bank_of=None, bank_normalize=True):
        from .. import ops
        stages = [getattr(self, nm) for nm in self.res_layers[:last + 1]]
        probe = x
        if (self.pool is None and x.is_cuda and x.dtype == torch.float32 and self.conv1.conv.out_channels % 32 == 0
                and all(self._split_stage_ok(st, probe) for st in stages)):
            N, dev = x.shape[0], x.device
            cache = self.__dict__.setdefault("_split_cache", {})
            if self.arith != "bf16x3" and self._scales(dev) is None and "_calib" not in self.__dict__:
                self.calibrate(None if self.calibration == "canonical" else x, last, device=dev)
            self._touch_workspace_shape((N, x.shape[2], x.shape[3], dev))
            n_lanes = 1 if N <= 2 else max(1, min(int(self.split_lanes), N))
            main = torch.cuda.current_stream(dev)
            c1 = self.conv1.conv
            stem7 = None
            f_stem = self._format_plan(last)["stem"]
            s_stem = (self._scales(dev) or {}).get(("stem",), 0) if f_stem != ops.ACT_BF16X2 else 0
            calib = self.__dict__.get("_calib")
            if self._stem7_ok():
                if ("stem7", dev) not in cache:
                    cache[("stem7", dev)] = ops.prepare_stem7(c1.weight.detach(), self.conv1.bn)
                    self._cache_filled(dev)
                stem7 = cache[("stem7", dev)]
                x = x.contiguous()
            x_cl = None if stem7 else x.contiguous(memory_format=torch.channels_last)
            if n_lanes > 1:
                skey = ("streams", dev, n_lanes)
                if skey not in cache:
                    cache[skey] = [torch.cuda.Stream(dev, priority=int(getattr(self, "lane_priority", 0))) for _ in range(n_lanes)]
                streams = cache[skey]
                for s in streams:
                    s.wait_stream(main)
            else:
                streams = [main]
            whole = bool(n_lanes > 1 and self.layer1_whole_batch and last >= 1 and calib is None and 0 not in fresh
                         and all(self._is_conv64(b.conv1) and self._is_conv64(b.conv2) for b in stages[0]))
            lane_streams = [main] if whole else streams
            lanes = []
            for li, s in enumerate(lane_streams):
                lo, hi = (0, N) if whole else (li * N // n_lanes, (li + 1) * N // n_lanes)
                with torch.cuda.stream(s):
                    if stem7:
                        H, W, C0 = (x.shape[2] - 1) // 2 + 1, (x.shape[3] - 1) // 2 + 1, 64
                        if self._identity_from_split(stages[0][0]):
                            sb = self._split_buffers(("stem",), N, C0, H, W, dev, ("s_x",))
                            t = None
                        else:
                            sb = self._split_buffers(("stem",), N, C0, H, W, dev, ("s_x", "f_x"))
                            t = sb["f_x"][lo:hi]
                        ops.stem7_split(x[lo:hi], stem7[0], stem7[1], True, out_split=sb["s_x"][lo:hi], out_f32=t, out_fmt=f_stem,
                                        out_scale_log2=s_stem, overflow=cache.get(("overflow", dev)))
                    else:
                        assert f_stem == ops.ACT_BF16X2
                        t = self._miopen_nhwc(("stem",), self.conv1, x_cl[lo:hi])
                        _, H, W, C0 = t.shape
                        sb = self._split_buffers(("stem",), N, C0, H, W, dev, ("s_x",))
                        ops.nhwc_to_split(t, sb["s_x"][lo:hi], relu=True)
                    if calib is not None:
                        calib[("stem",)] = torch.maximum(calib.get(("stem",), torch.zeros((), device=dev)),
                                                         sb["s_x"][lo:hi].view(torch.bfloat16)[..., :32].abs().amax().float())
                lanes.append(dict(split=sb["s_x"][lo:hi], f32=t, H=H, W=W, lo=lo, hi=hi, N=N, need_split=True, fmt=f_stem, scale=s_stem))
            fulls = []
            call = dict(main=main, streams=streams, fresh=tuple(fresh), out={}, last=last, bank_of=bank_of, bank_normalize=bool(bank_normalize))
            for i in range(last + 1):
                need_f32 = True
                if i < last and i not in call["fresh"]:
                    nb = stages[i + 1][0]
                    st = nb.conv1.conv.stride
                    need_f32 = nb.downsample is None or not (st == (1, 1) or (st == (2, 2) and self.use_s2_conv))
                if whole and i == 0:
                    one = self._stage_split(0, dict(lanes[0], need_split=True, need_f32=need_f32), call)
                    fulls.append(one["full"])
                    for s in streams:
                        s.wait_stream(main)
                    lanes = []
                    for li in range(n_lanes):
                        lo, hi = li * N // n_lanes, (li + 1) * N // n_lanes
                        lanes.append(dict(one, split=one["split"][lo:hi], f32=None if one["f32"] is None else one["f32"][lo:hi], lo=lo, hi=hi))
                    continue
                for li, s in enumerate(streams):
                    with torch.cuda.stream(s):
                        lanes[li] = self._stage_split(i, dict(lanes[li], need_split=i < last, need_f32=need_f32), call)
                fulls.append(lanes[0]["full"])
            if post is not None:
                for ln, s in zip(lanes, streams):
                    if ln.get("banked"):
                        continue
                    with torch.cuda.stream(s):
                        post(ln["f32"], ln["lo"], ln["hi"], ln["f32"].shape[-1], ln["H"], ln["W"])
            if n_lanes > 1:
                for s in streams:
                    main.wait_stream(s)
            outs = [f.permute(0, 3, 1, 2) for f in fulls]
            return outs[:-1], fulls[-1], True, lanes[0]["H"], lanes[0]["W"]
        x = self.conv1(x)
        if self.pool is not None:
            x = self.pool(x)
        outs = []
        for st in stages:
            x = st(x)
            outs.append(x)
        return outs[:-1], x, False, x.shape[-2], x.shape[-1]

    def forward(self, x, out_idx=None):
        want = tuple(out_idx) if out_idx is not None else self.out_indices
        last = max(want)
        earlier, y, nhwc, H, W = self._trunk(x, last, fresh=want)
        if nhwc:
            y = y.permute(0, 3, 1, 2)
        stage_out = earlier + [y]
        outs = [stage_out[i] for i in want]
        return outs[0] if len(outs) == 1 else tuple(outs)

    use_graph = "auto"
    graph_auto_max_px = 300_000

    def forward_hwc(self, x, normalize: bool = True, split_if=None, split_fmt: str = "bf16", out=None):
        want = self.use_graph is True or (self.use_graph == "auto" and x.dim() == 4 and x.shape[0] * x.shape[2] * x.shape[3] <= self.graph_auto_max_px)
        if not (want and x.is_cuda and not self.training and x.dtype == torch.float32) or torch.cuda.is_current_stream_capturing():
            return self.forward_hwc_eager(x, normalize, split_if, split_fmt, out)
        cache = self.__dict__.setdefault("_split_cache", {})
        sig = (self.arith, self.split_lanes, self.use_conv64, self.use_stem7, self.use_s2_conv, self.conv64_f16f8, self.res_from_split,
               self.use_split_conv, self.fuse_bank, self.fold_projection, self.layer1_whole_batch, tuple(self.out_indices))
        key = ("graph", tuple(x.shape), x.device, bool(normalize), split_fmt, split_if is not None, sig)
        ent = cache.get(key)
        if ent is None:
            cache[key] = "warm"
            return self.forward_hwc_eager(x, normalize, split_if, split_fmt, out)
        if ent == "warm":
            if self._scales(x.device) is None and self.arith != "bf16x3":
                return self.forward_hwc_eager(x, normalize, split_if, split_fmt, out)
            static_in = torch.empty_like(x)
            static_in.copy_(x)
            self.forward_hwc_eager(static_in, normalize, split_if, split_fmt, None)
            torch.cuda.synchronize(x.device)
            g = torch.cuda.CUDAGraph()
            _CAPTURING[0] = True
            try:
                with torch.cuda.graph(g):
                    o, H, W = self.forward_hwc_eager(static_in, normalize, split_if, split_fmt, None)
            finally:
                _CAPTURING[0] = False
            ent = cache[key] = (g, static_in, o, H, W)
        g, static_in, o, H, W = ent
        static_in.copy_(x)
        g.replay()
        if out is not None and tuple(out.shape) == tuple(o.shape) and out.dtype == o.dtype:
            out.copy_(o)
            return out, H, W
        return o.clone(), H, W

    def forward_hwc_eager(self, x, normalize: bool = True, split_if=None, split_fmt: str = "bf16", out=None):
        from .. import ops
        assert len(self.out_indices) == 1
        box = {}

        def ensure_out(C, H, W):
            if "out" not in box:
                as_split = bool(split_if is not None and split_if(C, H, W))
                shape = (x.shape[0], H * W, 4 if split_fmt == "f16f6x" else 2, C) if as_split else (x.shape[0], H * W, C)
                dtype = torch.int16 if as_split else torch.float32
                if out is not None and tuple(out.shape) == shape and out.dtype == dtype and out.is_contiguous() and out.device == x.device:
                    box["out"] = out
                else:
                    with torch.cuda.stream(main):
                        box["out"] = torch.empty(shape, device=x.device, dtype=dtype)
                torch.cuda.current_stream(x.device).wait_stream(main)
                box["split"] = as_split
            elif torch.cuda.current_stream(x.device) != main:
                torch.cuda.current_stream(x.device).wait_stream(main)

        def post(y_slice, lo, hi, C, H, W):
            ensure_out(C, H, W)
            ops.normalize_nhwc(y_slice, normalize, split=split_fmt if box["split"] else False, out=box["out"][lo:hi])

        def bank_of(lo, hi, C, H, W):
            if not (self.fuse_bank and split_fmt in ("f16f6", "f16f6x") and C == 256 and split_if is not None and split_if(C, H, W)):
                return None
            ensure_out(C, H, W)
            return box["out"][lo:hi] if box["split"] else None

        main = torch.cuda.current_stream(x.device) if x.is_cuda else None
        _, y, nhwc, H, W = self._trunk(x, self.out_indices[0], post=post, bank_of=bank_of, bank_normalize=normalize)
        if nhwc:
            return box["out"], H, W
        C = y.shape[1]
        as_split = bool(split_if is not None and split_if(C, H, W))
        f = ops.normalize_to_hwc(y.float(), normalize, pad=True)
        splitter = {"f16": ops.split_f16x2, "f16f6": ops.split_f16f6p, "f16f6x": ops.split_f16f6x}.get(split_fmt, ops.split_bf16)
        return (splitter(f) if as_split and f.shape[-1] == C else f), H, W


def torchvision_key(name: str) -> str:
    mod, _, leaf = name.rpartition(".")
    owner, _, part = mod.rpartition(".")
    if part not in ("conv", "bn"):
        return name
    if "downsample" in owner:
        return f"{owner}.{0 if part == 'conv' else 1}.{leaf}"
    return f"{owner if part == 'conv' else owner.replace('conv', 'bn')}.{leaf}"


def load_torchvision_checkpoint(module: nn.Module, filename_or_state):
    sd = torch.load(filename_or_state, map_location="cpu") if isinstance(filename_or_state, str) else filename_or_state
    if isinstance(sd, dict) and "state_dict" in sd:
        sd = sd["state_dict"]
    own = module.state_dict()
    used = set()
    with torch.no_grad():
        for k, v in own.items():
            tv = torchvision_key(k)
            if tv in sd:
                v.copy_(sd[tv])
                used.add(tv)
            elif not k.endswith("num_batches_tracked"):
                raise KeyError(f"torchvision checkpoint has no '{tv}' (for '{k}')")
    if hasattr(module, "reset_split_cache"):
        module.reset_split_cache()
    return sorted(set(sd) - used)


_PREFIXES = (r"^module\.", r"^backbone\.", r"^encoder\.", r"^backbone_fine\.")


def load_checkpoint(module: nn.Module, filename_or_state, strict: bool = False, prefixes: Sequence[str] = _PREFIXES):
    sd = torch.load(filename_or_state, map_location="cpu") if isinstance(filename_or_state, str) else filename_or_state
    if isinstance(sd, dict) and "state_dict" in sd:
        sd = sd["state_dict"]
    own = module.state_dict()
    out = {}
    for k, v in sd.items():
        kk = k
        if kk not in own:
            for p in prefixes:
                k2 = re.sub(p, "", kk)
                if k2 != kk and (k2 in own or not strict):
                    kk = k2
                    if kk in own:
                        break
        out[kk] = v
    return module.load_state_dict({k: v for k, v in out.items() if k in own} if not strict else out, strict=strict)
```

fgvc_amd/ops.py:

```python
from __future__ import annotations

import ctypes as C
import functools
import math
from dataclasses import dataclass
from typing import Optional, Tuple

import torch

from . import _lib
from ._lib import NO_LIMIT, PAIR_MASKED, WEIGHT_COSINE, WEIGHT_RAW, WEIGHT_SOFTMAX


@dataclass(frozen=True)
class MaskSpec:
    r2max: int = NO_LIMIT
    ry: int = NO_LIMIT
    rx: int = NO_LIMIT

    @property
    def is_none(self) -> bool:
        return self.r2max >= NO_LIMIT and self.ry >= NO_LIMIT and self.rx >= NO_LIMIT

    @staticmethod
# ... 718 lines not shown
        return packed, bias, e
    if fmt == ACT_F16F6:
        return _f16f6_slots(h, l, "h").contiguous().view(torch.int16), bias, e
    h8 = (h.float() * 2.0 ** -F8_AW).clamp(-448.0, 448.0).to(torch.float8_e4m3fn)
    l8 = (l * 2.0 ** F8_BW).clamp(-448.0, 448.0).to(torch.float8_e4m3fn)
    packed = torch.cat([h.contiguous().view(torch.uint8), h8.view(torch.uint8), l8.view(torch.uint8)], dim=-1).contiguous()
    return packed.view(torch.int16), bias, e


def prepare_conv64(weight: torch.Tensor, bn: "torch.nn.BatchNorm2d") -> Tuple[torch.Tensor, torch.Tensor]:
    assert tuple(weight.shape) == (64, 64, 3, 3)
    packed, bias = prepare_conv_split(weight, bn)
    v = packed.view(9, 2, 2, 32, 2, 2, 2, 8)
    v = v.permute(2, 0, 1, 5, 4, 6, 3, 7).contiguous()
    return v.view(2, 9, 2, 2, 2, 64, 8), bias


def prepare_conv64_f16(weight: torch.Tensor, bn: "torch.nn.BatchNorm2d") -> Tuple[torch.Tensor, torch.Tensor, int]:
    assert tuple(weight.shape) == (64, 64, 3, 3)
    packed, bias, e = prepare_conv_split_f16(weight, bn, ACT_F16F8)
    rows = packed.view(torch.uint8).view(9, 2, 2, 32, 128)
    hpart = rows[..., :64].reshape(9, 2, 2, 32, 2, 2, 16)
    f16 = hpart.permute(2, 0, 1, 4, 5, 3, 6)
    h8 = rows[..., 64:96].reshape(9, 2, 2, 32, 2, 16)
    l8 = rows[..., 96:128].reshape(9, 2, 2, 32, 2, 16)
    x = torch.stack([h8, l8], dim=-2).permute(2, 0, 1, 4, 3, 5, 6)
    out = torch.cat([f16.reshape(2, 9, 2, 2048), x.reshape(2, 9, 2, 2048)], dim=-1).contiguous()
    return out.view(torch.int16), bias, e


def prepare_conv_s2(weight: torch.Tensor, bn: "torch.nn.BatchNorm2d") -> Tuple[torch.Tensor, torch.Tensor]:
    packed, bias = prepare_conv_split(weight, bn)
    T, nch, Cout, _ = packed.shape
    assert Cout % 32 == 0
    v = packed.view(T, nch, Cout // 32, 32, 2, 2, 2, 8)
    v = v.permute(0, 1, 2, 4, 5, 6, 3, 7).contiguous()
    return v.view(T, nch, Cout // 32, 4, 64, 8), bias


def prepare_stem7(weight: torch.Tensor, bn: "torch.nn.BatchNorm2d") -> Tuple[torch.Tensor, torch.Tensor]:
    Cout, Cin, KS, _ = weight.shape
    assert (Cout, Cin, KS) == (64, 3, 7)
    scale = (bn.weight / torch.sqrt(bn.running_var + bn.eps)).float()
    w = weight.float() * scale.view(-1, 1, 1, 1)
    bias = (bn.bias - bn.running_mean * scale).float().contiguous()
    k = torch.zeros((Cout, 7, 8, 4), device=w.device, dtype=torch.float32)
    k[:, :, :7, :3] = w.permute(0, 2, 3, 1)
    k = k.reshape(2, 32, 7, 2, 2, 8)
    k = k.permute(2, 3, 0, 4, 1, 5).contiguous()
    hi, lo = _split_pair(k)
    packed = torch.stack([hi, lo], dim=3).contiguous()
    return packed.view(torch.int16).view(7, 2, 2, 2, 64, 8), bias


def alloc_split_nhwc(N: int, C: int, H: int, W: int, device) -> torch.Tensor:
    Hp, Wp = conv_pad_dims(H, W)
    return torch.zeros((N, Hp, Wp, C // 32, 64), device=device, dtype=torch.int16)


def alloc_nhwc(N: int, C: int, H: int, W: int, device) -> torch.Tensor:
    return torch.empty((N, H, W, C), device=device, dtype=torch.float32)


def nhwc_to_split(x: torch.Tensor, out: torch.Tensor, relu: bool = False) -> torch.Tensor:
    x = _chk(x, torch.float32, "x")
    N, H, W, C = x.shape
    Hp, Wp = conv_pad_dims(H, W)
    assert out.shape == (N, Hp, Wp, C // 32, 64) and out.dtype == torch.int16 and out.is_contiguous()
    _lib.call("fgvc_nhwc_to_split_f32", _ptr(x), _ptr(out), N, C, H, W, Hp, Wp, int(relu), _stream(x))
    return out


def nchw_to_split_nhwc(x: torch.Tensor, out: Optional[torch.Tensor] = None, out_f32: Optional[torch.Tensor] = None,
                       want_split: bool = True) -> Optional[torch.Tensor]:
    x = _chk(x, torch.float32, "x")
    N, C, H, W = x.shape
    if out is None and want_split:
        out = alloc_split_nhwc(N, C, H, W, x.device)
    Hp, Wp = conv_pad_dims(H, W)
    if out is not None:
        assert out.shape == (N, Hp, Wp, C // 32, 64) and out.dtype == torch.int16 and out.is_contiguous()
    if out_f32 is not None:
        assert out_f32.shape == (N, H, W, C) and out_f32.dtype == torch.float32 and out_f32.is_contiguous()
    _lib.call("fgvc_nchw_to_split_nhwc_f32", _ptr(x), _ptr(out), _ptr(out_f32), N, C, H, W, Hp, Wp, _stream(x))
    return out


def conv_split(x_split: torch.Tensor, w: torch.Tensor, bias: torch.Tensor, H: int, W: int, relu: bool,
               residual: Optional[torch.Tensor] = None, out_split: Optional[torch.Tensor] = None,
               out_f32: Optional[torch.Tensor] = None, in_fmt: int = ACT_BF16X2, in_scale_log2: int = 0,
               out_fmt: int = ACT_BF16X2, out_scale_log2: int = 0, overflow: Optional[torch.Tensor] = None,
               x2_split: Optional[torch.Tensor] = None, w2: Optional[torch.Tensor] = None) -> None:
    x_split, w = _chk(x_split, torch.int16, "x_split"), _chk(w, torch.int16, "w")
    bias = _chk(bias, torch.float32, "bias")
    N, Hp, Wp, nch, _ = x_split.shape
    taps, nch_w, Cout, _ = w.shape
    assert nch_w == nch and taps in (1, 9) and bias.shape == (Cout,)
    for t, dt, shape in ((residual, torch.float32, (N, H, W, Cout)), (out_f32, torch.float32, (N, H, W, Cout)),
                         (out_split, torch.int16, (N, Hp, Wp, Cout // 32, 64))):
        if t is not None:
            assert t.dtype == dt and tuple(t.shape) == shape and t.is_contiguous() and t.device == x_split.device, "conv_split buffer"
    if out_fmt != ACT_BF16X2 and out_split is not None:
        assert overflow is not None and overflow.dtype == torch.int32 and overflow.device == x_split.device
    if x2_split is not None:
        x2_split, w2 = _chk(x2_split, torch.int16, "x2_split"), _chk(w2, torch.int16, "w2")
        assert taps == 9 and Cout == 256, "conv_split: a second input goes with the 3 x 3 form of 256 output channels"
        assert tuple(x2_split.shape[:3]) == (N, Hp, Wp) and x2_split.shape[4] == 64 and tuple(w2.shape) == (1, x2_split.shape[3], Cout, 64)
        _lib.call("fgvc_conv_split_proj_fmt_f32", _ptr(x_split), _ptr(w), _ptr(x2_split), _ptr(w2), _ptr(bias), _ptr(residual), _ptr(out_split),
                  _ptr(out_f32), N, H, W, Hp, Wp, nch * 32, x2_split.shape[3] * 32, int(relu), int(in_fmt), int(in_scale_log2), int(out_fmt),
                  int(out_scale_log2), _ptr(overflow), _stream(x_split))
        return
    _lib.call("fgvc_conv_split_fmt_f32", _ptr(x_split), _ptr(w), _ptr(bias), _ptr(residual), _ptr(out_split), _ptr(out_f32),
              N, H, W, Hp, Wp, nch * 32, Cout, 3 if taps == 9 else 1, int(relu), int(in_fmt), int(in_scale_log2), int(out_fmt),
              int(out_scale_log2), _ptr(overflow), _stream(x_split))


def conv_split_to_bank(x_split: torch.Tensor, w: torch.Tensor, bias: torch.Tensor, H: int, W: int, relu: bool, bank: torch.Tensor,
                       residual: Optional[torch.Tensor] = None, in_fmt: int = ACT_BF16X2, in_scale_log2: int = 0,
                       normalize: bool = True) -> torch.Tensor:
    x_split, w = _chk(x_split, torch.int16, "x_split"), _chk(w, torch.int16, "w")
    bias = _chk(bias, torch.float32, "bias")
    N, Hp, Wp, nch, _ = x_split.shape
    taps, nch_w, Cout, _ = w.shape
    assert nch_w == nch and taps == 9 and bias.shape == (Cout,) and Cout == 256, "conv_split_to_bank: a 3 x 3 convolution with 256 output channels"
    assert bank.dtype == torch.int16 and tuple(bank.shape) in ((N, H * W, 2, 256), (N, H * W, 4, 256)) and bank.is_contiguous() and bank.device == x_split.device
    if residual is not None:
        assert residual.dtype == torch.float32 and tuple(residual.shape) == (N, H, W, Cout) and residual.is_contiguous()
    _lib.call("fgvc_conv_split_bank_f16f6x_f32" if bank.shape[2] == 4 else "fgvc_conv_split_bank_f16f6p_f32", _ptr(x_split), _ptr(w), _ptr(bias), _ptr(residual), _ptr(bank), N, H, W, Hp, Wp,
              nch * 32, 3, int(relu), int(in_fmt), int(in_scale_log2), int(normalize), _stream(x_split))
    return bank


def conv64_split(x_split: torch.Tensor, w: torch.Tensor, bias: torch.Tensor, H: int, W: int, relu: bool,
                 residual: Optional[torch.Tensor] = None, out_split: Optional[torch.Tensor] = None,
                 out_f32: Optional[torch.Tensor] = None, residual_split: Optional[torch.Tensor] = None,
                 in_fmt: int = ACT_BF16X2, in_scale_log2: int = 0, out_fmt: int = ACT_BF16X2, out_scale_log2: int = 0,
                 overflow: Optional[torch.Tensor] = None) -> None:
    x_split = _chk(x_split, torch.int16, "x_split")
    N, Hp, Wp, nch, _ = x_split.shape
    assert nch == 2 and bias.shape == (64,)
    assert tuple(w.shape) == ((2, 9, 2, 2, 2, 64, 8) if in_fmt == ACT_BF16X2 else (2, 9, 2, 2048)), "conv64_split weights / in_fmt"
    assert residual is None or residual_split is None, "one residual, f32 or split"
    for t, dt, shape in ((residual, torch.float32, (N, H, W, 64)), (out_f32, torch.float32, (N, H, W, 64)),
                         (out_split, torch.int16, (N, Hp, Wp, 2, 64)), (residual_split, torch.int16, (N, Hp, Wp, 2, 64))):
        if t is not None:
            assert t.dtype == dt and tuple(t.shape) == shape and t.is_contiguous() and t.device == x_split.device, "conv64_split buffer"
    _lib.call("fgvc_conv64_split_fmt_f32", _ptr(x_split), _ptr(w), _ptr(bias), _ptr(residual), _ptr(residual_split), _ptr(out_split),
              _ptr(out_f32), N, H, W, Hp, Wp, int(relu), int(in_fmt), int(in_scale_log2), int(out_fmt), int(out_scale_log2),
              _ptr(overflow), _stream(x_split))


def conv_s2_split(x_split: torch.Tensor, w: torch.Tensor, bias: torch.Tensor, H: int, W: int, relu: bool,
                  out_split: Optional[torch.Tensor] = None, out_f32: Optional[torch.Tensor] = None, out_fmt: int = ACT_BF16X2,
                  out_scale_log2: int = 0, overflow: Optional[torch.Tensor] = None) -> None:
    x_split = _chk(x_split, torch.int16, "x_split")
    N, Hp, Wp, nch, _ = x_split.shape
    taps, nch_w, n_ct = w.shape[:3]
    Cout = n_ct * 32
    assert tuple(w.shape[3:]) == (4, 64, 8) and nch_w == nch and taps in (1, 9) and bias.shape == (Cout,)
    Ho, Wo = (H - 1) // 2 + 1, (W - 1) // 2 + 1
    Hop, Wop = conv_pad_dims(Ho, Wo)
    if out_split is not None:
        assert out_split.dtype == torch.int16 and tuple(out_split.shape) == (N, Hop, Wop, Cout // 32, 64) and out_split.is_contiguous()
    if out_f32 is not None:
        assert out_f32.dtype == torch.float32 and tuple(out_f32.shape) == (N, Ho, Wo, Cout) and out_f32.is_contiguous()
    if out_fmt != ACT_BF16X2 and out_split is not None:
        assert overflow is not None and overflow.dtype == torch.int32 and overflow.device == x_split.device
    _lib.call("fgvc_conv_s2_split_fmt_f32", _ptr(x_split), _ptr(w), _ptr(bias), _ptr(out_split), _ptr(out_f32), N, H, W, Hp, Wp,
              nch * 32, Cout, 3 if taps == 9 else 1, Hop, Wop, int(relu), int(out_fmt), int(out_scale_log2), _ptr(overflow),
              _stream(x_split))


def stem7_split(x: torch.Tensor, w: torch.Tensor, bias: torch.Tensor, relu: bool = True,
                out_split: Optional[torch.Tensor] = None, out_f32: Optional[torch.Tensor] = None, out_fmt: int = ACT_BF16X2,
                out_scale_log2: int = 0, overflow: Optional[torch.Tensor] = None) -> None:
    x = _chk(x, torch.float32, "x")
    N, C, H, W = x.shape
    assert C == 3 and x.is_contiguous() and tuple(w.shape) == (7, 2, 2, 2, 64, 8) and bias.shape == (64,)
    Ho, Wo = (H - 1) // 2 + 1, (W - 1) // 2 + 1
    Hop, Wop = conv_pad_dims(Ho, Wo)
    if out_split is not None:
        assert out_split.dtype == torch.int16 and tuple(out_split.shape) == (N, Hop, Wop, 2, 64) and out_split.is_contiguous()
    if out_f32 is not None:
        assert out_f32.dtype == torch.float32 and tuple(out_f32.shape) == (N, Ho, Wo, 64) and out_f32.is_contiguous()
    _lib.call("fgvc_stem7_split_fmt_f32", _ptr(x), _ptr(w), _ptr(bias), _ptr(out_split), _ptr(out_f32), N, H, W, Hop, Wop,
              int(relu), int(out_fmt), int(out_scale_log2), _ptr(overflow), _stream(x))


def normalize_nhwc(x: torch.Tensor, normalize: bool = True, split=False, out: Optional[torch.Tensor] = None) -> torch.Tensor:
    fmt = "bf16" if split is True else split
    assert fmt in (False, "bf16", "f16", "f16f6", "f16f6x")
    x = _chk(x, torch.float32, "x")
    N, H, W, C = x.shape
    shape, dt = ((N, H * W, 4 if fmt == "f16f6x" else 2, C), torch.int16) if split else ((N, H * W, C), torch.float32)
    if out is None:
        out = torch.empty(shape, device=x.device, dtype=dt)
    else:
        assert tuple(out.shape) == shape and out.dtype == dt and out.is_contiguous() and out.device == x.device
    if fmt in ("f16f6", "f16f6x"):
        assert C == 256
        _lib.call(f"fgvc_normalize_split_{fmt}p_nhwc_f32" if fmt == "f16f6" else "fgvc_normalize_split_f16f6x_nhwc_f32", _ptr(x), _ptr(out), N, C, H, W,
                  int(normalize), _stream(x))
        return out
    _lib.call("fgvc_normalize_split_f16x2_nhwc_f32" if fmt == "f16" else "fgvc_normalize_split_nhwc_f32", _ptr(x),
              _ptr(None if split else out), _ptr(out if split else None), N, C, H, W, int(normalize), _stream(x))
    return out


def unsplit_f16x2(split: torch.Tensor) -> torch.Tensor:
    v = split.view(torch.float16).float()
    return (v[..., 0, :] + v[..., 1, :]) * (1.0 / 16384.0)


def unsplit_act(split: torch.Tensor, fmt: int, scale_log2: int = 0) -> torch.Tensor:
    n5 = split.shape
    if fmt == ACT_BF16X2:
        v = split.view(torch.bfloat16).float()
        return (v[..., :32] + v[..., 32:]).reshape(*n5[:3], -1)
    b = split.contiguous().view(torch.uint8).reshape(*n5[:4], 128)
    h = b[..., :64].contiguous().view(torch.float16).float()
    if fmt == ACT_F16X2:
        l = b[..., 64:].contiguous().view(torch.float16).float()
    elif fmt == ACT_F16F6:
        l = _e2m3_decode(torch.cat([b[..., 64:80], b[..., 96:104]], dim=-1), b[..., 104])
    else:
        l = b[..., 64:96].contiguous().view(torch.float8_e4m3fn).float() * 2.0 ** -F8_BX
    return ((h + l) * 2.0 ** -scale_log2).reshape(*n5[:3], -1)


def unsplit_bf16(split: torch.Tensor) -> torch.Tensor:
    v = split.view(torch.bfloat16).float()
    return v[..., 0, :] + v[..., 1, :]


def gaussian_labels(points: torch.Tensor, Hf: int, Wf: int, stride: int, sigma: float = 6.0,
                    out: Optional[torch.Tensor] = None) -> torch.Tensor:
    points = _chk(points.to(torch.float32), torch.float32, "points")
    P = points.shape[0]
    if out is None:
        out = torch.empty((Hf * Wf, P), device=points.device, dtype=torch.float32)
    _lib.call("fgvc_gaussian_labels_f32", _ptr(points), P, Hf, Wf, stride, float(sigma), _ptr(out), _stream(points))
    return out


def softargmax_top5(labels: torch.Tensor, Hf: int, Wf: int, h: int, w: int,
                    gauss_points: Optional[torch.Tensor] = None, sigma: float = 6.0) -> torch.Tensor:
    labels = _chk(labels, torch.float32, "labels")
    n, P = labels.shape[0], labels.shape[2]
    assert labels.shape[1] == Hf * Wf
    if gauss_points is not None:
        gauss_points = _chk(gauss_points.to(torch.float32), torch.float32, "gauss_points")
        assert gauss_points.shape == (P, 2)
    coords = torch.empty((n, P, 2), device=labels.device, dtype=torch.float64)
    ws_bytes = _lib.load().fgvc_softargmax_workspace_bytes(n, P)
    ws = torch.empty((max(ws_bytes, 4) + 3) // 4, device=labels.device, dtype=torch.float32)
    _lib.call("fgvc_softargmax_top5_f32", _ptr(labels), n, Hf, Wf, P, h, w, _ptr(gauss_points), float(sigma),
              _ptr(coords), _ptr(ws), _stream(labels))
    return coords



def pil_nearest_index(n_in: int, n_out: int) -> torch.Tensor:
    a, xo, out = n_in / n_out, n_in / n_out * 0.5, []
    for _ in range(n_out):
        out.append(min(int(xo), n_in - 1))
        xo += a
    return torch.tensor(out, dtype=torch.int64)


def seg_max_label(seg_map: torch.Tensor, Hf: int, Wf: int, out: Optional[torch.Tensor] = None) -> torch.Tensor:
    seg_map = _chk(seg_map, torch.uint8, "seg_map")
    hp, wp = seg_map.shape
    if out is None:
        out = torch.empty((1,), device=seg_map.device, dtype=torch.int32)
    _lib.call("fgvc_seg_max_label_u8", _ptr(seg_map), hp, wp, Hf, Wf, _ptr(out), _stream(seg_map))
    return out


def seg_onehot_labels(seg_map: torch.Tensor, Hf: int, Wf: int, C: int, out: Optional[torch.Tensor] = None) -> torch.Tensor:
    seg_map = _chk(seg_map, torch.uint8, "seg_map")
    hp, wp = seg_map.shape
    if out is None:
        out = torch.empty((Hf * Wf, C), device=seg_map.device, dtype=torch.float32)
    else:
        assert out.is_contiguous() and out.shape == (Hf * Wf, C) and out.dtype == torch.float32
    _lib.call("fgvc_seg_onehot_labels_u8", _ptr(seg_map), hp, wp, Hf, Wf, C, _ptr(out), _stream(seg_map))
    return out


def seg_hard_onehot(labels: torch.Tensor, out: Optional[torch.Tensor] = None) -> torch.Tensor:
    labels = _chk(labels, torch.float32, "labels")
    C = labels.shape[-1]
    if out is None:
        out = torch.empty_like(labels)
    else:
        assert out.is_contiguous() and out.shape == labels.shape and out.dtype == torch.float32
    _lib.call("fgvc_seg_hard_onehot_f32", _ptr(labels), labels.numel() // C, C, _ptr(out), _stream(labels))
    return out


def seg_readout(labels: torch.Tensor, Hf: int, Wf: int, pad_shape: Tuple[int, int], pad: Tuple[int, int, int, int],
                out_shape: Tuple[int, int], norm: bool = True, out: Optional[torch.Tensor] = None) -> torch.Tensor:
    labels = _chk(labels, torch.float32, "labels")
    n, C = labels.shape[0], labels.shape[2]
    assert labels.shape[1] == Hf * Wf
    (hp, wp), (lw, uw, lh, uh), (h0, w0) = pad_shape, pad, out_shape
    if out is None:
        out = torch.empty((n, h0, w0), device=labels.device, dtype=torch.uint8)
    else:
        assert out.is_contiguous() and out.shape == (n, h0, w0) and out.dtype == torch.uint8
    ws = torch.empty((max(_lib.load().fgvc_seg_readout_workspace_bytes(n, C), 4) + 3) // 4, device=labels.device, dtype=torch.float32)
    _lib.call("fgvc_seg_readout_u8", _ptr(labels), n, Hf, Wf, C, hp, wp, lh, lw, hp - lh - uh, wp - lw - uw, h0, w0, int(bool(norm)),
              _ptr(out), _ptr(ws), _stream(labels))
    return out



def _heat(heat: torch.Tensor) -> torch.Tensor:
    if not heat.is_cuda:
        raise _lib.FgvcHipError("heat must be on the GPU (fgvc_amd has no CPU path)")
# ... 229 lines not shown
```

include/fgvc_hip.h:

```cpp
#ifndef FGVC_HIP_H
#define FGVC_HIP_H

#include <stddef.h>
#include <stdint.h>

#ifdef __cplusplus
extern "C" {
#endif

#define FGVC_OK 0
#define FGVC_ERR_INVALID_ARG 1
#define FGVC_ERR_UNSUPPORTED 2
#define FGVC_ERR_LAUNCH 3

#define FGVC_NO_LIMIT 0x3fffffff

#define FGVC_PAIR_MASKED 1

#define FGVC_WEIGHT_SOFTMAX 0
#define FGVC_WEIGHT_COSINE 1
#define FGVC_WEIGHT_RAW 2

const char* fgvc_version(void);
const char* fgvc_last_error(void);
// ... 15 lines not shown
                         float* score_out, void* stream);
int fgvc_pair_topk_f16x3_runs(const uint16_t* qsplit, const uint16_t* ksplit, const int32_t* pairs, int n_pairs, int C, int Hq, int Wq,
                              int Hk, int Wk, int r2max, int ry, int rx, int topk, int all_masked, const int32_t* runs, int n_runs,
                              int32_t* idx_out, float* score_out, void* stream);
int fgvc_pair_topk_f16x3_timed_out(void);

int fgvc_split_f16f6p(const float* feat, uint8_t* rows, int64_t n_pixels, int C, void* stream);
int fgvc_pair_topk_f16f6(const uint8_t* qsplit, const uint8_t* ksplit, const int32_t* pairs, int n_pairs, int C, int Hq, int Wq, int Hk,
                         int Wk, int r2max, int ry, int rx, int topk, int all_masked, int32_t* idx_out, float* score_out, void* stream);
int fgvc_pair_topk_f16f6_runs(const uint8_t* qsplit, const uint8_t* ksplit, const int32_t* pairs, int n_pairs, int C, int Hq, int Wq,
                              int Hk, int Wk, int r2max, int ry, int rx, int topk, int all_masked, const int32_t* runs, int n_runs,
                              int32_t* idx_out, float* score_out, void* stream);
int fgvc_split_f16f6x(const float* feat, uint8_t* rows, int64_t n_pixels, int C, void* stream);
int fgvc_pair_topk_f16f6x(const uint8_t* qrows, const uint8_t* krows, const int32_t* pairs, int n_pairs, int C, int Hq, int Wq, int Hk,
                          int Wk, int r2max, int ry, int rx, int topk, int all_masked, int32_t* idx_out, float* score_out, void* stream);
int fgvc_pair_topk_f16f6x_runs(const uint8_t* qrows, const uint8_t* krows, const int32_t* pairs, int n_pairs, int C, int Hq, int Wq,
                               int Hk, int Wk, int r2max, int ry, int rx, int topk, int all_masked, const int32_t* runs, int n_runs,
                               int32_t* idx_out, float* score_out, void* stream);
int fgvc_pair_topk_f16x3_probe(int64_t* out32);

int fgvc_merge_topk_f32(const int32_t* pair_idx, const float* pair_score, const int32_t* slot_pair,
                        int n_out, int T, int HWq, int HWk, int topk, float temperature,
                        int weight_mode, int32_t* idx_out, float* logit_out, float* weight_out,
                        void* stream);

size_t fgvc_merge_refine_workspace_bytes(int n_out, int HWq);
int fgvc_merge_refine_topk_f32(const int32_t* pair_idx, const float* pair_score, const int32_t* slot_pair, const int32_t* pairs,
                               const void* q_exact, int64_t q_frame_bytes, int q_row_bytes, const void* k_exact, int64_t k_frame_bytes,
                               int k_row_bytes, int n_out, int T, int Hq, int Wq, int Hk, int Wk, int C, int topk, float temperature,
                               int weight_mode, float eps, int r2max, int ry, int rx, int32_t* idx_out, float* logit_out,
                               float* weight_out, void* workspace, void* stream);

int fgvc_propagate_topk_f32(const float* labels, const int32_t* slot_frame, int T,
                            const int32_t* idx, const float* weight, int Hq, int Wq, int Hk, int Wk,
                            int P, int topk, int window_L, float* out, void* stream);

int fgvc_corr_volume_f32(const float* qfeat, const float* kfeat, int C, int HWq, int HWk,
                         float temperature, float* vol, void* stream);
int fgvc_split_bf16(const float* feat, uint16_t* hi_lo , int64_t n_pixels,
                    int C, void* stream);
int fgvc_corr_volume_bf16x3(const uint16_t* q_hi_lo, const uint16_t* k_hi_lo, int C, int HWq, int HWk,
                            float temperature, float* vol, void* stream);
int fgvc_corr_volume_bf16(const uint16_t* q_hi_lo, const uint16_t* k_hi_lo, int C, int HWq, int HWk,
                          float temperature, float* vol, void* stream);

int fgvc_split_f16f8(const float* feat, uint8_t* out, int64_t n_pixels, int C, void* stream);
int fgvc_corr_volume_f16f8(const uint8_t* q_split, const uint8_t* k_split, int C, int HWq, int HWk,
                           float temperature, float* vol, void* stream);

int fgvc_split_f16f6(const float* feat, uint8_t* out, int64_t n_pixels, int C, void* stream);
int fgvc_corr_volume_f16f6(const uint8_t* q_split, const uint8_t* k_split, int C, int HWq, int HWk,
                           float temperature, float* vol, void* stream);

int fgvc_debug_store_sweep_f32(float* buf, int64_t n_floats, int nontemporal, void* stream);

int fgvc_dense_attend_splits(int HWq, int HWk);
int fgvc_dense_attend_f32(const float* vol, const float* labels, int Hq, int Wq, int Hk, int Wk, int P, int masked,
                          int r2max, int ry, int rx, int weight_mode, int first, float* state, int nsplit, void* stream);
int fgvc_dense_attend_finish_f32(const float* state, int nsplit, int HWq, int P, int weight_mode, float* out, void* stream);

int fgvc_dense_kth_f32(const float* aff, int HWk, int HWq, int k, float* part, int nsplit, float* thr, void* stream);
int fgvc_dense_propagate_f32(const float* aff, const float* labels, int HWk, int HWq, int P, const float* thr, float* state,
                             int nsplit, float* out, void* stream);

int fgvc_local_corr_topk_f32(const float* qfeat, const float* kfeat, const int32_t* pairs, int n_slots,
                             int C, int H, int W, int R, int topk, float temperature,
                             int32_t* pair_idx_ws, float* pair_score_ws,
                             int32_t* idx_out, float* logit_out, float* weight_out, void* stream);
int fgvc_local_corr_topk_f16x3(const uint16_t* qsplit, const uint16_t* ksplit, const int32_t* pairs, int n_slots,
                               int C, int H, int W, int R, int topk, float temperature,
                               int32_t* pair_idx_ws, float* pair_score_ws,
                               int32_t* idx_out, float* logit_out, float* weight_out, void* stream);

int fgvc_local_merge_plan_f32(const int32_t* pair_idx, const float* pair_score, int n_pairs, const int32_t* slot_pair, int n_rows,
                              int max_slots, int H, int W, int R, int topk, float temperature, int32_t* idx_out, float* logit_out,
                              float* weight_out, void* stream);

int fgvc_topk_coord_f32(const int32_t* idx, const float* weight, int H, int W, int R, int topk, int scale,
                        float* out, void* stream);
int fgvc_topk_coord_rows_f32(const int32_t* idx, const float* weight, int rows, int H, int W, int R, int topk, int scale,
                             float* out, void* stream);

int fgvc_cycle_chase_f32(const float* fields, const float* traj, const float* start_xy, int n, int P, int H, int W, int scale,
                         float* back_out, float* err_out, void* stream);

int fgvc_frames_rgb8_to_lab_f32(const uint8_t* frames, int T, int h0, int w0, int64_t stride_t, int64_t stride_y, int64_t stride_x,
                                int64_t stride_c, int h, int w, int pad_left, int pad_right, int pad_top, int pad_bottom, float* out,
                                void* stream);

int fgvc_jf_counts_u8(const uint8_t* gt, const uint8_t* pred, int T, int h, int w, int n_objects, int radius, int64_t* counts, void* stream);
int fgvc_jf_tile_rows(void);

int fgvc_render_frames_u8(const uint8_t* frames, int64_t frames_stride_t, int64_t frames_stride_y, uint8_t* out, int64_t out_stride_t,
                          int64_t out_stride_y, int T, int h, int w, const uint8_t* ids, int64_t ids_stride_t, int64_t ids_stride_y,
                          const uint8_t* palette, int alpha, int contour, const double* tracks, int64_t tracks_stride_p,
                          int64_t tracks_stride_t, const uint8_t* visibles, int64_t visibles_stride_p, int64_t visibles_stride_t,
                          const uint8_t* colors, int P, int radius, const double* icon, void* stream);
int fgvc_render_tile_rows(void);
int fgvc_render_tile_cols(void);

int fgvc_c2f_refine_f32(const int32_t* coarse_arg, const float* qfine, const float* kfine,
                        const float* vfine, int T, int H, int W, int scale, int Cf, int P, int Rf,
                        int topk, float temperature, float* out, int32_t* idx_out, float* logit_out,
                        void* stream);
int fgvc_c2f_refine_mode_f32(const int32_t* coarse_arg, const float* qfine, const float* kfine, const float* vfine, int T,
                             int H, int W, int scale, int Cf, int P, int Rf, int topk, float temperature, int weight_mode,
                             float* out, int32_t* idx_out, float* logit_out, void* stream);

int fgvc_bn_act_f32(const float* x, const float* residual, const float* mean, const float* var,
                    const float* gamma, const float* beta, float eps, int relu, float* out, int N, int C,
                    int HW, void* stream);

int fgvc_nchw_to_split_nhwc_f32(const float* in , uint16_t* out_split ,
                                float* out_f32 , int N, int C, int H, int W,
                                int Hp, int Wp, void* stream);
int fgvc_nhwc_to_split_f32(float* x, uint16_t* out_split, int N, int C, int H, int W, int Hp, int Wp, int relu,
                           void* stream);
int fgvc_conv_split_f32(const uint16_t* x, const uint16_t* w, const float* bias, const float* residual,
                        uint16_t* y_split, float* y_f32, int N, int H, int W, int Hp, int Wp, int Cin, int Cout,
                        int KS, int relu, void* stream);
#define FGVC_ACT_BF16X2 0
#define FGVC_ACT_F16F8 1
#define FGVC_ACT_F16X2 2
#define FGVC_ACT_F16F6 3
int fgvc_conv_split_fmt_f32(const uint16_t* x, const uint16_t* w, const float* bias, const float* residual,
                            uint16_t* y_split, float* y_f32, int N, int H, int W, int Hp, int Wp, int Cin, int Cout,
                            int KS, int relu, int in_fmt, int in_scale_log2, int out_fmt, int out_scale_log2, int* overflow,
                            void* stream);
int fgvc_conv_split_proj_fmt_f32(const uint16_t* x, const uint16_t* w, const uint16_t* x2, const uint16_t* w2, const float* bias,
                                 const float* residual, uint16_t* y_split, float* y_f32, int N, int H, int W, int Hp, int Wp, int Cin,
                                 int Cin2, int relu, int in_fmt, int in_scale_log2, int out_fmt, int out_scale_log2, int* overflow,
                                 void* stream);
int fgvc_conv_split_bank_f16f6p_f32(const uint16_t* x, const uint16_t* w, const float* bias, const float* residual, void* bank,
                                    int N, int H, int W, int Hp, int Wp, int Cin, int KS, int relu, int in_fmt, int in_scale_log2,
                                    int normalize, void* stream);
int fgvc_conv_split_bank_f16f6x_f32(const uint16_t* x, const uint16_t* w, const float* bias, const float* residual, void* bank,
                                    int N, int H, int W, int Hp, int Wp, int Cin, int KS, int relu, int in_fmt, int in_scale_log2,
                                    int normalize, void* stream);
int fgvc_conv64_split_f32(const uint16_t* x, const uint16_t* w, const float* bias, const float* residual, uint16_t* y_split,
                          float* y_f32, int N, int H, int W, int Hp, int Wp, int relu, void* stream);
int fgvc_conv64_split_fmt_f32(const uint16_t* x, const uint16_t* w, const float* bias, const float* residual,
                              const uint16_t* residual_split, uint16_t* y_split, float* y_f32, int N, int H, int W, int Hp, int Wp,
                              int relu, int in_fmt, int in_scale_log2, int out_fmt, int out_scale_log2, int* overflow, void* stream);
int fgvc_conv64_probe(int64_t* out32);
int fgvc_conv64_split_res_f32(const uint16_t* x, const uint16_t* w, const float* bias, const float* residual,
                              const uint16_t* residual_split, uint16_t* y_split, float* y_f32, int N, int H, int W, int Hp, int Wp,
                              int relu, void* stream);
int fgvc_conv_s2_split_f32(const uint16_t* x, const uint16_t* w, const float* bias, uint16_t* y_split, float* y_f32, int N,
                           int H, int W, int Hp, int Wp, int Cin, int Cout, int KS, int Hop, int Wop, int relu,
                           void* stream);
int fgvc_conv_s2_split_fmt_f32(const uint16_t* x, const uint16_t* w, const float* bias, uint16_t* y_split, float* y_f32, int N,
                               int H, int W, int Hp, int Wp, int Cin, int Cout, int KS, int Hop, int Wop, int relu, int out_fmt,
                               int out_scale_log2, int* overflow, void* stream);
int fgvc_stem7_split_f32(const float* x, const uint16_t* w, const float* bias, uint16_t* y_split, float* y_f32, int N, int H,
                         int W, int Hop, int Wop, int relu, void* stream);
int fgvc_stem7_split_fmt_f32(const float* x, const uint16_t* w, const float* bias, uint16_t* y_split, float* y_f32, int N, int H,
                             int W, int Hop, int Wop, int relu, int out_fmt, int out_scale_log2, int* overflow, void* stream);
int fgvc_normalize_nhwc_f32(const float* in, float* out, int N, int C, int H, int W, int normalize, void* stream);
int fgvc_normalize_split_nhwc_f32(const float* in, float* out_f32, uint16_t* out_split, int N, int C, int H, int W,
                                  int normalize, void* stream);
int fgvc_normalize_split_f16x2_nhwc_f32(const float* in, float* out_f32, uint16_t* out_split, int N, int C, int H, int W,
                                        int normalize, void* stream);
int fgvc_normalize_split_f16f6p_nhwc_f32(const float* in, uint8_t* rows, int N, int C, int H, int W, int normalize, void* stream);
int fgvc_normalize_split_f16f6x_nhwc_f32(const float* in, uint8_t* rows, int N, int C, int H, int W, int normalize, void* stream);

int fgvc_gaussian_labels_f32(const float* points, int P, int Hf, int Wf, int stride, float sigma,
                             float* out, void* stream);

size_t fgvc_softargmax_workspace_bytes(int n_frames, int P);
int fgvc_softargmax_top5_f32(const float* labels, int n_frames, int Hf, int Wf, int P, int h, int w,
                             const float* gauss_points, float sigma, double* coords, void* workspace,
                             void* stream);

int fgvc_seg_max_label_u8(const uint8_t* map, int hp, int wp, int Hf, int Wf, int32_t* out, void* stream);
int fgvc_seg_onehot_labels_u8(const uint8_t* map, int hp, int wp, int Hf, int Wf, int C, float* out, void* stream);

int fgvc_seg_hard_onehot_f32(const float* in, int rows, int C, float* out, void* stream);

size_t fgvc_seg_readout_workspace_bytes(int n, int C);
int fgvc_seg_readout_u8(const float* labels, int n, int Hf, int Wf, int C, int hp, int wp, int top, int left, int h, int w, int h0,
                        int w0, int norm, uint8_t* masks, void* workspace, void* stream);

int fgvc_seg_soft_labels_f32(const float* map, int K, int hm, int wm, int hp, int wp, int top, int left, int Hf, int Wf, float* out,
                             void* stream);
int fgvc_seg_soft_labels_f64(const double* map, int K, int hm, int wm, int hp, int wp, int top, int left, int Hf, int Wf, float* out,
                             void* stream);

size_t fgvc_heatmap_coords_workspace_bytes(int T, int K);
int fgvc_heatmap_coords_f32(const float* bank, const void* map0, int map0_f64, int T, int Hf, int Wf, int K, int hm, int wm, int hp,
                            int wp, int top, int left, int h0, int w0, int f64_arith, double* coords, void* workspace, void* stream);

int fgvc_softmap_readout_f32(const float* bank, const void* map0, int map0_f64, int T, int Hf, int Wf, int K, int hm, int wm, int hp,
                             int wp, int top, int left, int h0, int w0, int f_begin, int f_end, int out_f64, void* out, void* stream);

#ifdef __cplusplus
}
#endif
#endif
```

Baseline: 1910.

## Fuse strided 1x1 downsample projection into the 3x3 stride-2 conv kernel

The 1x1 stride-2 downsample projection now runs inside the 3x3 stride-2 conv kernel. It reuses the centre tap of the staged input patch with a second accumulator and weight set, so the input activations are read once instead of twice and one launch per downsample block goes away. The cost is a second 32-element accumulator pair per wave, which adds register pressure. The launch bound is also raised from 2 to 4 workgroups per CU, which may limit registers further or cause spills. The output path is moved into a shared helper so it can write both outputs.

```diff
diff --git a/fgvc_amd/_lib.py b/fgvc_amd/_lib.py
--- a/fgvc_amd/_lib.py
+++ b/fgvc_amd/_lib.py
@@ -50,6 +50,7 @@
     "fgvc_conv64_split_fmt_f32": (_i, [_p, _p, _p, _p, _p, _p, _p, _i, _i, _i, _i, _i, _i, _i, _i, _i, _i, _p, _p]),
     "fgvc_conv_s2_split_f32": (_i, [_p, _p, _p, _p, _p, _i, _i, _i, _i, _i, _i, _i, _i, _i, _i, _i, _p]),
     "fgvc_conv_s2_split_fmt_f32": (_i, [_p, _p, _p, _p, _p, _i, _i, _i, _i, _i, _i, _i, _i, _i, _i, _i, _i, _i, _p, _p]),
+    "fgvc_conv_s2_split_proj_fmt_f32": (_i, [_p, _p, _p, _p, _p, _p, _p, _p, _i, _i, _i, _i, _i, _i, _i, _i, _i, _i, _i, _i, _i, _i, _i, _p, _p]),
     "fgvc_stem7_split_f32": (_i, [_p, _p, _p, _p, _p, _i, _i, _i, _i, _i, _i, _p]),
     "fgvc_stem7_split_fmt_f32": (_i, [_p, _p, _p, _p, _p, _i, _i, _i, _i, _i, _i, _i, _i, _p, _p]),
     "fgvc_nhwc_to_split_f32": (_i, [_p, _p, _i, _i, _i, _i, _i, _i, _i, _p]),
diff --git a/fgvc_amd/csrc/capi.hip b/fgvc_amd/csrc/capi.hip
--- a/fgvc_amd/csrc/capi.hip
+++ b/fgvc_amd/csrc/capi.hip
@@ -51,7 +51,7 @@
                       int, int, int, int, int, int, int, int, int*, hipStream_t, unsigned char* y_bank = nullptr, int bank_normalize = 1, const uint16_t* x2 = nullptr,
                       const uint16_t* w2 = nullptr, int Cin2 = 0, int bank_row_bytes = 1024);
 int conv_s2_launch(const uint16_t*, const uint16_t*, const float*, uint16_t*, float*, int, int, int, int, int, int, int, int, int,
-                   int, int, int, int, int*, hipStream_t);
+                   int, int, int, int, int*, const uint16_t*, const float*, float*, int, hipStream_t);
 int conv64_launch(const uint16_t*, const uint16_t*, const float*, const float*, const uint16_t*, uint16_t*, float*, int, int, int, int, int, int,
                   int, int, int, int, int*, hipStream_t);
 int stem7_launch(const float*, const uint16_t*, const float*, uint16_t*, float*, int, int, int, int, int, int, int, int, int, int, int*,
@@ -826,6 +826,14 @@
 int fgvc_conv_s2_split_fmt_f32(const uint16_t* x, const uint16_t* w, const float* bias, uint16_t* y_split, float* y_f32, int N,
                                int H, int W, int Hp, int Wp, int Cin, int Cout, int KS, int Hop, int Wop, int relu, int out_fmt,
                                int out_scale_log2, int* overflow, void* stream) {
+  return fgvc_conv_s2_split_proj_fmt_f32(x, w, bias, y_split, y_f32, nullptr, nullptr, nullptr, N, H, W, Hp, Wp, Cin, Cout, KS, Cout, Hop, Wop,
+                                         relu, 0, out_fmt, out_scale_log2, overflow, stream);
+}
+
+int fgvc_conv_s2_split_proj_fmt_f32(const uint16_t* x, const uint16_t* w, const float* bias, uint16_t* y_split, float* y_f32,
+                                    const uint16_t* w2, const float* bias2, float* y2_f32, int N, int H, int W, int Hp, int Wp, int Cin,
+                                    int Cout, int KS, int Cout2, int Hop, int Wop, int relu, int relu2, int out_fmt, int out_scale_log2,
+                                    int* overflow, void* stream) {
   FGVC_REQUIRE(x && w && bias && (y_split || y_f32), FGVC_ERR_INVALID_ARG, "fgvc_conv_s2_split_f32: null pointer");
   FGVC_REQUIRE(out_fmt >= 0 && out_fmt <= 3 && out_scale_log2 > -100 && out_scale_log2 < 100, FGVC_ERR_INVALID_ARG, "fgvc_conv_s2_split_fmt_f32: bad output format / scale");
   FGVC_REQUIRE(out_fmt == FGVC_ACT_BF16X2 || !y_split || overflow, FGVC_ERR_INVALID_ARG, "fgvc_conv_s2_split_fmt_f32: an f16-format output needs the overflow word");
@@ -840,9 +848,16 @@
   FGVC_REQUIRE(aligned16(x) && aligned16(w) && aligned16(bias) && aligned16(y_split) && aligned16(y_f32),
                FGVC_ERR_INVALID_ARG, "fgvc_conv_s2_split_f32: 16-byte alignment required");
   FGVC_REQUIRE((const void*)x != (const void*)y_split, FGVC_ERR_INVALID_ARG, "fgvc_conv_s2_split_f32: in-place not supported");
+  if (w2 || bias2 || y2_f32) {
+    FGVC_REQUIRE(w2 && bias2 && y2_f32, FGVC_ERR_INVALID_ARG, "fgvc_conv_s2_split_proj_fmt_f32: null pointer (w2, bias2 and y2_f32 go together)");
+    FGVC_REQUIRE(KS == 3, FGVC_ERR_UNSUPPORTED, "fgvc_conv_s2_split_proj_fmt_f32: the projection rides in the 3x3 kernel only (KS = %d)", KS);
+    FGVC_REQUIRE(Cout2 == Cout, FGVC_ERR_UNSUPPORTED, "fgvc_conv_s2_split_proj_fmt_f32: the projection's Cout=%d differs from the convolution's %d", Cout2, Cout);
+    FGVC_REQUIRE(aligned16(w2) && aligned16(bias2) && aligned16(y2_f32), FGVC_ERR_INVALID_ARG, "fgvc_conv_s2_split_proj_fmt_f32: 16-byte alignment required");
+    FGVC_REQUIRE((const void*)y2_f32 != (const void*)y_f32, FGVC_ERR_INVALID_ARG, "fgvc_conv_s2_split_proj_fmt_f32: the two f32 outputs must differ");
+  }
   if (N == 0) return FGVC_OK;
   return conv_s2_launch(x, w, bias, y_split, y_f32, N, Hp, Wp, Cin, Cout, KS, Ho, Wo, Hop, Wop, relu, out_fmt, out_scale_log2, overflow,
-                        (hipStream_t)stream);
+                        w2, bias2, y2_f32, relu2, (hipStream_t)stream);
 }
 
 int fgvc_stem7_split_f32(const float* x, const uint16_t* w, const float* bias, uint16_t* y_split, float* y_f32, int N, int H,
diff --git a/fgvc_amd/csrc/conv_s2.hip b/fgvc_amd/csrc/conv_s2.hip
--- a/fgvc_amd/csrc/conv_s2.hip
+++ b/fgvc_amd/csrc/conv_s2.hip
@@ -14,6 +14,10 @@
   float out_scale;
   int out_fmt;
   int* overflow;
+  const uint16_t* w2;
+  const float* bias2;
+  float* y2_f32;
+  int relu2;
 };
 
 
@@ -30,8 +34,102 @@
 constexpr int S2_CPG = 1;
 constexpr int S2_RS = 144;
 
-template <int KS>
-__global__ __launch_bounds__(64 * S2_NW, 2) void conv_s2_kernel(ConvS2Params p) {
+__device__ __forceinline__ void s2_wave_sync() { asm volatile("s_waitcnt lgkmcnt(0)" ::: "memory"); }
+
+struct S2Wave {
+  int nimg, y0, x0, half, co_w;
+};
+
+__device__ __forceinline__ void s2_write_rows(const ConvS2Params& p, const S2Wave& wv, const f32x16 (&acc)[2], const f32x4 (&bias_v)[4], int relu,
+                                              float* y_f32, uint16_t* y_split, int out_fmt, float out_scale, unsigned char* tile, int lane) {
+  const int n = lane & 31, h = lane >> 5;
+  const int x0 = wv.x0, co_w = wv.co_w;
+  const int mv_row = lane >> 3, mv_col = (lane & 7) * 16;
+#pragma unroll
+  for (int b = 0; b < 2; ++b) {
+    const int y = wv.y0 + wv.half * 2 + b;
+    if (y >= p.Ho) continue;
+    f32x4 v[4];
+#pragma unroll
+    for (int g = 0; g < 4; ++g) {
+      const f32x4 bv = bias_v[g];
+      v[g] = {acc[b][4 * g + 0] + bv.x, acc[b][4 * g + 1] + bv.y, acc[b][4 * g + 2] + bv.z, acc[b][4 * g + 3] + bv.w};
+      if (relu) {
+        v[g].x = fmaxf(v[g].x, 0.f); v[g].y = fmaxf(v[g].y, 0.f); v[g].z = fmaxf(v[g].z, 0.f); v[g].w = fmaxf(v[g].w, 0.f);
+      }
+    }
+    if (y_f32) {
+#pragma unroll
+      for (int g = 0; g < 4; ++g) *reinterpret_cast<f32x4*>(tile + n * S2_RS + (8 * g + 4 * h) * 4) = v[g];
+      s2_wave_sync();
+      unsigned char* dst = reinterpret_cast<unsigned char*>(y_f32 + (((size_t)wv.nimg * p.Ho + y) * p.Wo + x0) * p.Cout + co_w);
+#pragma unroll
+      for (int i = 0; i < 4; ++i) {
+        const int row = i * 8 + mv_row;
+        if (x0 + row < p.Wo)
+          *reinterpret_cast<uint4*>(dst + (size_t)row * p.Cout * 4 + mv_col) =
+              *reinterpret_cast<const uint4*>(tile + row * S2_RS + mv_col);
+      }
+      s2_wave_sync();
+    }
+    if (y_split) {
+      if (out_fmt == 0) {
+#pragma unroll
+        for (int g = 0; g < 4; ++g) {
+          const f32x4 x = v[g];
+          ushort4 hv, lv;
+          split_bf16_4(x, hv, lv);
+          unsigned char* o = tile + n * S2_RS + (8 * g + 4 * h) * 2;
+          *reinterpret_cast<ushort4*>(o) = hv;
+          *reinterpret_cast<ushort4*>(o + 64) = lv;
+        }
+      } else if (out_fmt == 3) {
+        bool ovf = false;
+        uint2 hw[4];
+        fgvc_i32x4 main6, tail6;
+        split_f16f6_chunk(v, out_scale, h, hw, main6, tail6, ovf);
+        unsigned char* o = tile + n * S2_RS;
+#pragma unroll
+        for (int g = 0; g < 4; ++g) *reinterpret_cast<uint2*>(o + (8 * g + 4 * h) * 2) = hw[g];
+        *reinterpret_cast<fgvc_i32x4*>(o + 80 - 16 * h) = main6;
+        *reinterpret_cast<fgvc_i32x4*>(o + 112 - 16 * h) = tail6;
+        if (__builtin_amdgcn_ballot_w64(ovf && x0 + n < p.Wo) != 0ull && lane == 0) atomicOr(p.overflow, 1);
+      } else {
+        bool ovf = false;
+#pragma unroll
+        for (int g = 0; g < 4; ++g) {
+          uint2 hw, lw;
+          uint32_t l8, h8;
+          split_f16_4(v[g], out_scale, hw, l8, h8, lw, ovf);
+          unsigned char* o = tile + n * S2_RS;
+          *reinterpret_cast<uint2*>(o + (8 * g + 4 * h) * 2) = hw;
+          if (out_fmt == 1) {
+            *reinterpret_cast<uint32_t*>(o + 64 + 8 * g + 4 * h) = l8;
+            *reinterpret_cast<uint32_t*>(o + 96 + 8 * g + 4 * h) = h8;
+          } else {
+            *reinterpret_cast<uint2*>(o + 64 + (8 * g + 4 * h) * 2) = lw;
+          }
+        }
+        if (__builtin_amdgcn_ballot_w64(ovf && x0 + n < p.Wo) != 0ull && lane == 0) atomicOr(p.overflow, 1);
+      }
+      s2_wave_sync();
+      const size_t pix0 = ((size_t)wv.nimg * p.Hop + (y + 1)) * p.Wop + (x0 + 1);
+      unsigned char* dst = reinterpret_cast<unsigned char*>(y_split) + (pix0 * (p.Cout / 32) + (co_w >> 5)) * 128;
+#pragma unroll
+      for (int i = 0; i < 4; ++i) {
+        const int row = i * 8 + mv_row;
+        if (x0 + row < p.Wo)
+          *reinterpret_cast<uint4*>(dst + (size_t)row * p.Cout * 4 + mv_col) =
+              *reinterpret_cast<const uint4*>(tile + row * S2_RS + mv_col);
+      }
+      s2_wave_sync();
+    }
+  }
+}
+
+template <int KS, bool PROJ = false>
+__global__ __launch_bounds__(64 * S2_NW, 4) void conv_s2_kernel(ConvS2Params p) {
+  static_assert(!PROJ || (KS == 3 && S2_CPG == 1), "the projection rides in the 3x3 kernel, one chunk staged at a time");
   constexpr int T = KS * KS;
   constexpr int NR = KS == 3 ? 2 * S2_TR + 1 : S2_TR;
   constexpr int NC = KS == 3 ? 65 : 32;
@@ -41,7 +139,6 @@
   constexpr int SMEMB = S2_CPG * CHUNKB > S2_NW * 32 * S2_RS ? S2_CPG * CHUNKB : S2_NW * 32 * S2_RS;
   static_assert(SMEMB <= 79 * 1024, "LDS: two workgroups per CU");
   __shared__ __attribute__((aligned(16))) unsigned char smem[SMEMB];
-  auto wave_sync = [&]() { asm volatile("s_waitcnt lgkmcnt(0)" ::: "memory"); };
 
   const int tid = threadIdx.x, lane = tid & 63;
   const int wave = __builtin_amdgcn_readfirstlane(tid >> 6);
@@ -58,17 +155,20 @@
   const size_t pix_bytes_in = (size_t)nchunk * 128;
   const int d_row = lane >> 3, d_slot = lane & 7;
 
-  f32x16 acc[2];
+  f32x16 acc[2], acc2[2];
 #pragma unroll
   for (int b = 0; b < 2; ++b)
 #pragma unroll
-    for (int r = 0; r < 16; ++r) acc[b][r] = 0.f;
+    for (int r = 0; r < 16; ++r) acc[b][r] = acc2[b][r] = 0.f;
 
   const int n_ct = p.Cout / 32;
-  const uint16_t* wlane = p.w + (size_t)(active ? (co_w >> 5) : 0) * 2048 + lane * 8;
+  const uint32_t wlane = ((active ? (co_w >> 5) : 0) * 2048 + lane * 8) * 2;
   f32x4 bias_v[4];
-#pragma unroll
-  for (int g = 0; g < 4; ++g) bias_v[g] = *reinterpret_cast<const f32x4*>(p.bias + (active ? co_w : 0) + 8 * g + 4 * h);
+  auto load_bias = [&](f32x4* bv, const float* bias) {
+#pragma unroll
+    for (int g = 0; g < 4; ++g) bv[g] = *reinterpret_cast<const f32x4*>(bias + (active ? co_w : 0) + 8 * g + 4 * h);
+  };
+  if (!PROJ) load_bias(bias_v, p.bias);
 
   for (int cg = 0; cg < nchunk; cg += S2_CPG) {
     const int ncg = imin(S2_CPG, nchunk - cg);
@@ -95,129 +195,68 @@
 
     const int nit = ncg * T;
     bf16x8 a_cur[4], a_nxt[4];
-    auto load_a = [&](bf16x8* a, int it) {
+    auto load_a = [&](bf16x8* a, const uint16_t* wp) {
+      const unsigned char* src = reinterpret_cast<const unsigned char*>((p.debug & 8) ? p.w : wp) + wlane;
+#pragma unroll
+      for (int q = 0; q < 4; ++q) a[q] = *reinterpret_cast<const bf16x8*>(src + q * 1024);
+    };
+    auto w_of = [&](int it) {
       const int cc = it / T, t = it - cc * T;
-      const uint16_t* wp = wlane + ((size_t)t * nchunk + (cg + cc)) * n_ct * 2048;
-#pragma unroll
-      for (int q = 0; q < 4; ++q) a[q] = *reinterpret_cast<const bf16x8*>((p.debug & 8) ? wlane + q * 512 : wp + q * 512);
+      return p.w + ((size_t)t * nchunk + (cg + cc)) * n_ct * 2048;
     };
-    load_a(a_cur, 0);
-    for (int it = 0; it < nit; ++it) {
-      if (it + 1 < nit) load_a(a_nxt, it + 1);
-      __builtin_amdgcn_sched_barrier(0);
-      const int cc = it / T, t = it - cc * T;
-      const int dy = KS == 3 ? t / 3 : 0, dx = KS == 3 ? t - 3 * (t / 3) : 0;
+    auto tap = [&](f32x16 (&c)[2], int cc, int dy, int dx, int n) {
       const int mbase = KS == 3 ? (dx == 0 ? 0 : dx == 1 ? 33 : 1) : 0;
       const unsigned char* patch = smem + cc * CHUNKB;
 #pragma unroll
       for (int b = 0; b < 2; ++b) {
         const int r = half * 2 + b;
         const int e = (KS == 3 ? (2 * r + dy) : r) * NC + mbase + n;
+        const int a0 = s2_swz(e, h);
         bf16x8 xh[2], xl[2];
 #pragma unroll
         for (int s = 0; s < 2; ++s) {
-          xh[s] = *reinterpret_cast<const bf16x8*>(patch + s2_swz(e, 2 * s + h));
-          xl[s] = *reinterpret_cast<const bf16x8*>(patch + s2_swz(e, 4 + 2 * s + h));
+          xh[s] = *reinterpret_cast<const bf16x8*>(patch + (a0 ^ (32 * s)));
+          xl[s] = *reinterpret_cast<const bf16x8*>(patch + (a0 ^ (64 + 32 * s)));
         }
         if (p.debug & 2) {
-          acc[b][0] += (float)(xh[0][0] + xl[0][0] + xh[1][0] + xl[1][0] + a_cur[0][0] + a_cur[1][0] + a_cur[2][0] + a_cur[3][0]);
+          asm volatile("" ::"v"(xh[0]), "v"(xh[1]), "v"(xl[0]), "v"(xl[1]), "v"(a_cur[0]), "v"(a_cur[1]), "v"(a_cur[2]), "v"(a_cur[3]));
           continue;
         }
 #pragma unroll
         for (int s = 0; s < 2; ++s) {
-          acc[b] = __builtin_amdgcn_mfma_f32_32x32x16_bf16(a_cur[s], xh[s], acc[b], 0, 0, 0);
-          acc[b] = __builtin_amdgcn_mfma_f32_32x32x16_bf16(a_cur[2 + s], xh[s], acc[b], 0, 0, 0);
-          acc[b] = __builtin_amdgcn_mfma_f32_32x32x16_bf16(a_cur[s], xl[s], acc[b], 0, 0, 0);
-        }
-      }
+          c[b] = __builtin_amdgcn_mfma_f32_32x32x16_bf16(a_cur[s], xh[s], c[b], 0, 0, 0);
+          c[b] = __builtin_amdgcn_mfma_f32_32x32x16_bf16(a_cur[2 + s], xh[s], c[b], 0, 0, 0);
+          c[b] = __builtin_amdgcn_mfma_f32_32x32x16_bf16(a_cur[s], xl[s], c[b], 0, 0, 0);
+        }
+      }
+    };
+    load_a(a_cur, w_of(0));
+#pragma unroll 1
+    for (int it = 0; it < nit; ++it) {
+      if (it + 1 < nit) load_a(a_nxt, w_of(it + 1));
+      else if (PROJ) load_a(a_nxt, p.w2 + (size_t)cg * n_ct * 2048);
+      __builtin_amdgcn_sched_barrier(0);
+      const int cc = it / T, t = it - cc * T;
+      tap(acc, cc, KS == 3 ? t / 3 : 0, KS == 3 ? t - 3 * (t / 3) : 0, n);
 #pragma unroll
       for (int q = 0; q < 4; ++q) a_cur[q] = a_nxt[q];
     }
+    if (PROJ) {
+      int n_here = n;
+      asm volatile("" : "+v"(n_here));
+      tap(acc2, 0, 1, 1, n_here);
+    }
     __syncthreads();
   }
   if (!active || (p.debug & 4)) return;
 
   unsigned char* tile = smem + wave * (32 * S2_RS);
-  const int mv_row = lane >> 3, mv_col = (lane & 7) * 16;
-#pragma unroll
-  for (int b = 0; b < 2; ++b) {
-    const int y = y0 + half * 2 + b;
-    if (y >= p.Ho) continue;
-    f32x4 v[4];
-#pragma unroll
-    for (int g = 0; g < 4; ++g) {
-      const f32x4 bv = bias_v[g];
-      v[g] = {acc[b][4 * g + 0] + bv.x, acc[b][4 * g + 1] + bv.y, acc[b][4 * g + 2] + bv.z, acc[b][4 * g + 3] + bv.w};
-      if (p.relu) {
-        v[g].x = fmaxf(v[g].x, 0.f); v[g].y = fmaxf(v[g].y, 0.f); v[g].z = fmaxf(v[g].z, 0.f); v[g].w = fmaxf(v[g].w, 0.f);
-      }
-    }
-    if (p.y_f32) {
-#pragma unroll
-      for (int g = 0; g < 4; ++g) *reinterpret_cast<f32x4*>(tile + n * S2_RS + (8 * g + 4 * h) * 4) = v[g];
-      wave_sync();
-      unsigned char* dst = reinterpret_cast<unsigned char*>(p.y_f32 + (((size_t)nimg * p.Ho + y) * p.Wo + x0) * p.Cout + co_w);
-#pragma unroll
-      for (int i = 0; i < 4; ++i) {
-        const int row = i * 8 + mv_row;
-        if (x0 + row < p.Wo)
-          *reinterpret_cast<uint4*>(dst + (size_t)row * p.Cout * 4 + mv_col) =
-              *reinterpret_cast<const uint4*>(tile + row * S2_RS + mv_col);
-      }
-      wave_sync();
-    }
-    if (p.y_split) {
-      if (p.out_fmt == 0) {
-#pragma unroll
-        for (int g = 0; g < 4; ++g) {
-          const f32x4 x = v[g];
-          ushort4 hv, lv;
-          split_bf16_4(x, hv, lv);
-          unsigned char* o = tile + n * S2_RS + (8 * g + 4 * h) * 2;
-          *reinterpret_cast<ushort4*>(o) = hv;
-          *reinterpret_cast<ushort4*>(o + 64) = lv;
-        }
-      } else if (p.out_fmt == 3) {
-        bool ovf = false;
-        uint2 hw[4];
-        fgvc_i32x4 main6, tail6;
-        split_f16f6_chunk(v, p.out_scale, h, hw, main6, tail6, ovf);
-        unsigned char* o = tile + n * S2_RS;
-#pragma unroll
-        for (int g = 0; g < 4; ++g) *reinterpret_cast<uint2*>(o + (8 * g + 4 * h) * 2) = hw[g];
-        *reinterpret_cast<fgvc_i32x4*>(o + 80 - 16 * h) = main6;
-        *reinterpret_cast<fgvc_i32x4*>(o + 112 - 16 * h) = tail6;
-        if (__builtin_amdgcn_ballot_w64(ovf && x0 + n < p.Wo) != 0ull && lane == 0) atomicOr(p.overflow, 1);
-      } else {
-        bool ovf = false;
-#pragma unroll
-        for (int g = 0; g < 4; ++g) {
-          uint2 hw, lw;
-          uint32_t l8, h8;
-          split_f16_4(v[g], p.out_scale, hw, l8, h8, lw, ovf);
-          unsigned char* o = tile + n * S2_RS;
-          *reinterpret_cast<uint2*>(o + (8 * g + 4 * h) * 2) = hw;
-          if (p.out_fmt == 1) {
-            *reinterpret_cast<uint32_t*>(o + 64 + 8 * g + 4 * h) = l8;
-            *reinterpret_cast<uint32_t*>(o + 96 + 8 * g + 4 * h) = h8;
-          } else {
-            *reinterpret_cast<uint2*>(o + 64 + (8 * g + 4 * h) * 2) = lw;
-          }
-        }
-        if (__builtin_amdgcn_ballot_w64(ovf && x0 + n < p.Wo) != 0ull && lane == 0) atomicOr(p.overflow, 1);
-      }
-      wave_sync();
-      const size_t pix0 = ((size_t)nimg * p.Hop + (y + 1)) * p.Wop + (x0 + 1);
-      unsigned char* dst = reinterpret_cast<unsigned char*>(p.y_split) + (pix0 * (p.Cout / 32) + (co_w >> 5)) * 128;
-#pragma unroll
-      for (int i = 0; i < 4; ++i) {
-        const int row = i * 8 + mv_row;
-        if (x0 + row < p.Wo)
-          *reinterpret_cast<uint4*>(dst + (size_t)row * p.Cout * 4 + mv_col) =
-              *reinterpret_cast<const uint4*>(tile + row * S2_RS + mv_col);
-      }
-      wave_sync();
-    }
+  const S2Wave wv = {nimg, y0, x0, half, co_w};
+  if (PROJ) load_bias(bias_v, p.bias);
+  s2_write_rows(p, wv, acc, bias_v, p.relu, p.y_f32, p.y_split, p.out_fmt, p.out_scale, tile, lane);
+  if (PROJ) {
+    load_bias(bias_v, p.bias2);
+    s2_write_rows(p, wv, acc2, bias_v, p.relu2, p.y2_f32, nullptr, 0, 0.f, tile, lane);
   }
 }
 
@@ -226,16 +265,23 @@
 
 int conv_s2_launch(const uint16_t* x, const uint16_t* w, const float* bias, uint16_t* y_split, float* y_f32, int N, int Hp,
                    int Wp, int Cin, int Cout, int KS, int Ho, int Wo, int Hop, int Wop, int relu, int out_fmt, int out_scale_log2,
-                   int* overflow, hipStream_t s) {
+                   int* overflow, const uint16_t* w2, const float* bias2, float* y2_f32, int relu2, hipStream_t s) {
   ConvS2Params p;
   p.out_fmt = out_fmt; p.out_scale = ldexpf(1.0f, out_scale_log2); p.overflow = overflow;
   p.x = x; p.w = w; p.bias = bias; p.y_split = y_split; p.y_f32 = y_f32;
   p.N = N; p.Hp = Hp; p.Wp = Wp; p.Cin = Cin; p.Cout = Cout; p.Ho = Ho; p.Wo = Wo; p.Hop = Hop; p.Wop = Wop; p.relu = relu;
+  p.w2 = w2; p.bias2 = bias2; p.y2_f32 = y2_f32; p.relu2 = relu2;
   p.n_ty = cdiv(Ho, S2_TR); p.n_tx = cdiv(Wo, 32);
   p.debug = g_conv_s2_debug;
   dim3 grid(p.n_ty * p.n_tx * N, cdiv(Cout, 128));
-  if (KS == 3) conv_s2_kernel<3><<<grid, 64 * S2_NW, 0, s>>>(p);
-  else conv_s2_kernel<1><<<grid, 64 * S2_NW, 0, s>>>(p);
+  if (w2) {
+    FGVC_REQUIRE(KS == 3, FGVC_ERR_UNSUPPORTED, "fgvc_conv_s2_split_f32: the projection rides in the 3x3 kernel only (KS = %d)", KS);
+    conv_s2_kernel<3, true><<<grid, 64 * S2_NW, 0, s>>>(p);
+  } else if (KS == 3) {
+    conv_s2_kernel<3><<<grid, 64 * S2_NW, 0, s>>>(p);
+  } else {
+    conv_s2_kernel<1><<<grid, 64 * S2_NW, 0, s>>>(p);
+  }
   FGVC_CHECK_LAUNCH("fgvc_conv_s2_split_f32");
   return FGVC_OK;
 }
diff --git a/fgvc_amd/mmpt_api/backbones.py b/fgvc_amd/mmpt_api/backbones.py
--- a/fgvc_amd/mmpt_api/backbones.py
+++ b/fgvc_amd/mmpt_api/backbones.py
@@ -131,6 +131,7 @@
     use_split_conv = True
     arith = "f16f6"
     fold_projection = True
+    fuse_s2_projection = True
     layer1_whole_batch = True
     fuse_bank = True
 
@@ -450,10 +451,15 @@
                 H, W = (Hi - 1) // 2 + 1, (Wi - 1) // 2 + 1
                 bufs = self._split_buffers((si, bi), N, Cout, H, W, dev, ("s_a", "s_y", "f_y", "f_idt"))
                 buf = {k: v[lo:hi] for k, v in bufs.items()}
-                ops.conv_s2_split(cur["split"], wt["ds"][0], wt["ds"][1], Hi, Wi, relu=False, out_f32=buf["f_idt"])
                 idt = buf["f_idt"]
-                ops.conv_s2_split(cur["split"], wt["c1"][0], wt["c1"][1], Hi, Wi, relu=True, out_split=buf["s_a"], out_fmt=f_a,
-                                  out_scale_log2=s_a, overflow=ovf)
+                w1, wd = wt["c1"][0], wt["ds"][0]
+                if self.fuse_s2_projection and calib is None and w1.shape[0] == 9 and wd.shape[0] == 1 and wd.shape[2] == w1.shape[2]:
+                    ops.conv_s2_split(cur["split"], w1, wt["c1"][1], Hi, Wi, relu=True, out_split=buf["s_a"], out_fmt=f_a,
+                                      out_scale_log2=s_a, overflow=ovf, proj=(wd, wt["ds"][1], idt))
+                else:
+                    ops.conv_s2_split(cur["split"], wd, wt["ds"][1], Hi, Wi, relu=False, out_f32=idt)
+                    ops.conv_s2_split(cur["split"], w1, wt["c1"][1], Hi, Wi, relu=True, out_split=buf["s_a"], out_fmt=f_a,
+                                      out_scale_log2=s_a, overflow=ovf)
             elif blk.conv1.conv.stride != (1, 1):
                 x_cl = cur["f32"].permute(0, 3, 1, 2)
                 t1 = self._miopen_nhwc((si, bi, "c1"), blk.conv1, x_cl)
@@ -640,7 +646,7 @@
             return self.forward_hwc_eager(x, normalize, split_if, split_fmt, out)
         cache = self.__dict__.setdefault("_split_cache", {})
         sig = (self.arith, self.split_lanes, self.use_conv64, self.use_stem7, self.use_s2_conv, self.conv64_f16f8, self.res_from_split,
-               self.use_split_conv, self.fuse_bank, self.fold_projection, self.layer1_whole_batch, tuple(self.out_indices))
+               self.use_split_conv, self.fuse_bank, self.fold_projection, self.fuse_s2_projection, self.layer1_whole_batch, tuple(self.out_indices))
         key = ("graph", tuple(x.shape), x.device, bool(normalize), split_fmt, split_if is not None, sig)
         ent = cache.get(key)
         if ent is None:
diff --git a/fgvc_amd/ops.py b/fgvc_amd/ops.py
--- a/fgvc_amd/ops.py
+++ b/fgvc_amd/ops.py
@@ -894,13 +894,26 @@
 
 def conv_s2_split(x_split: torch.Tensor, w: torch.Tensor, bias: torch.Tensor, H: int, W: int, relu: bool,
                   out_split: Optional[torch.Tensor] = None, out_f32: Optional[torch.Tensor] = None, out_fmt: int = ACT_BF16X2,
-                  out_scale_log2: int = 0, overflow: Optional[torch.Tensor] = None) -> None:
-    x_split = _chk(x_split, torch.int16, "x_split")
+                  out_scale_log2: int = 0, overflow: Optional[torch.Tensor] = None,
+                  proj: Optional[Tuple[torch.Tensor, torch.Tensor, torch.Tensor]] = None, proj_relu: bool = False) -> None:
     N, Hp, Wp, nch, _ = x_split.shape
     taps, nch_w, n_ct = w.shape[:3]
     Cout = n_ct * 32
+    Ho, Wo = (H - 1) // 2 + 1, (W - 1) // 2 + 1
+    if proj is not None:
+        w2, bias2, out2 = proj
+        if taps != 9:
+            raise ValueError("conv_s2_split: a projection rides in the 3x3 form only (w has %d taps)" % taps)
+        if w2.dim() != 6 or tuple(w2.shape[:2]) != (1, nch) or tuple(w2.shape[3:]) != (4, 64, 8) or w2.dtype != torch.int16:
+            raise ValueError("conv_s2_split: proj weights must be prepare_conv_s2's 1x1 form (1, %d, Cout/32, 4, 64, 8) int16, got %s %s"
+                             % (nch, tuple(w2.shape), w2.dtype))
+        if w2.shape[2] != n_ct or tuple(bias2.shape) != (Cout,):
+            raise ValueError("conv_s2_split: the projection's Cout (%d, bias %s) differs from the convolution's %d"
+                             % (w2.shape[2] * 32, tuple(bias2.shape), Cout))
+        if out2.dtype != torch.float32 or tuple(out2.shape) != (N, Ho, Wo, Cout) or not out2.is_contiguous():
+            raise ValueError("conv_s2_split: proj output must be contiguous f32 %s" % ((N, Ho, Wo, Cout),))
+    x_split = _chk(x_split, torch.int16, "x_split")
     assert tuple(w.shape[3:]) == (4, 64, 8) and nch_w == nch and taps in (1, 9) and bias.shape == (Cout,)
-    Ho, Wo = (H - 1) // 2 + 1, (W - 1) // 2 + 1
     Hop, Wop = conv_pad_dims(Ho, Wo)
     if out_split is not None:
         assert out_split.dtype == torch.int16 and tuple(out_split.shape) == (N, Hop, Wop, Cout // 32, 64) and out_split.is_contiguous()
@@ -908,6 +921,13 @@
         assert out_f32.dtype == torch.float32 and tuple(out_f32.shape) == (N, Ho, Wo, Cout) and out_f32.is_contiguous()
     if out_fmt != ACT_BF16X2 and out_split is not None:
         assert overflow is not None and overflow.dtype == torch.int32 and overflow.device == x_split.device
+    if proj is not None:
+        w2, bias2, out2 = _chk(proj[0], torch.int16, "proj w2"), _chk(proj[1], torch.float32, "proj bias2"), proj[2]
+        assert out2.device == x_split.device
+        _lib.call("fgvc_conv_s2_split_proj_fmt_f32", _ptr(x_split), _ptr(w), _ptr(bias), _ptr(out_split), _ptr(out_f32), _ptr(w2), _ptr(bias2),
+                  _ptr(out2), N, H, W, Hp, Wp, nch * 32, Cout, 3, w2.shape[2] * 32, Hop, Wop, int(relu), int(proj_relu), int(out_fmt),
+                  int(out_scale_log2), _ptr(overflow), _stream(x_split))
+        return
     _lib.call("fgvc_conv_s2_split_fmt_f32", _ptr(x_split), _ptr(w), _ptr(bias), _ptr(out_split), _ptr(out_f32), N, H, W, Hp, Wp,
               nch * 32, Cout, 3 if taps == 9 else 1, Hop, Wop, int(relu), int(out_fmt), int(out_scale_log2), _ptr(overflow),
               _stream(x_split))
diff --git a/include/fgvc_hip.h b/include/fgvc_hip.h
--- a/include/fgvc_hip.h
+++ b/include/fgvc_hip.h
@@ -191,6 +191,10 @@
 int fgvc_conv_s2_split_fmt_f32(const uint16_t* x, const uint16_t* w, const float* bias, uint16_t* y_split, float* y_f32, int N,
                                int H, int W, int Hp, int Wp, int Cin, int Cout, int KS, int Hop, int Wop, int relu, int out_fmt,
                                int out_scale_log2, int* overflow, void* stream);
+int fgvc_conv_s2_split_proj_fmt_f32(const uint16_t* x, const uint16_t* w, const float* bias, uint16_t* y_split, float* y_f32,
+                                    const uint16_t* w2, const float* bias2, float* y2_f32, int N, int H, int W, int Hp, int Wp, int Cin,
+                                    int Cout, int KS, int Cout2, int Hop, int Wop, int relu, int relu2, int out_fmt, int out_scale_log2,
+                                    int* overflow, void* stream);
 int fgvc_stem7_split_f32(const float* x, const uint16_t* w, const float* bias, uint16_t* y_split, float* y_f32, int N, int H,
                          int W, int Hop, int Wop, int relu, void* stream);
 int fgvc_stem7_split_fmt_f32(const float* x, const uint16_t* w, const float* bias, uint16_t* y_split, float* y_f32, int N, int H,
```

New measurement: 1934, median of 6. 1.2% higher.
